# wuliwei9278/primalCR

Hardware: AMD Instinct MI355X
Metric: pairwise-comparisons/sec (higher is better)
Workload: dtype f32; 1 GPU; ml1m-shaped PrimalCR++ -k 100 -l 5000 (configs[1]); 6040 users x 3952 items, 939809 ratings, 131347247 ordered pairs; 1 step = 1 outer iteration (V step + U step); solver=PrimalCR++, rank=100, parallelism=user-sharded x1, accumulation=f64, storage=f32

## Files before the change

primalcr_amd/csrc/pcr_classes.h:

```cpp
#pragma once
#include <cstdio>
#include <cstring>

#include "pcr_dev.h"
#include "pcr_kernels.h"
#include "pcr_gram.h"

struct Bin {
    int block = 64;
    bool big = false;
    int K = 1;
    int ugrid = 0;
    int scratch_ofs = 0;
    int cap = 0;
    int limit = 0;
    int rcap = 0;
    int unr = 4;
    bool gram = false;
    int wcap = 0;
    int sym = 0;
    int max_lev = 0;
    int64_t nnz = 0;
    std::vector<int32_t> users;
    DBuf<int32_t> d_users;
};
static const int BIN_LIMIT[3] = {128, 512, 4096};
static const int BIN_BLOCK[4] = {64, 256, 512, 512};
static const int GRAM_DEFAULT_CAP = 0;

static void length_order(const std::vector<int64_t>& uptr, int64_t nu, std::vector<int32_t>& order) {
    order.resize((size_t)nu);
    int64_t maxlen = 0;
    for (int64_t u = 0; u < nu; ++u) maxlen = std::max(maxlen, uptr[u + 1] - uptr[u]);
    if (maxlen > ((int64_t)1 << 24)) {
        for (int64_t u = 0; u < nu; ++u) order[u] = (int32_t)u;
        std::stable_sort(order.begin(), order.end(), [&](int32_t a, int32_t b) { return (uptr[a + 1] - uptr[a]) > (uptr[b + 1] - uptr[b]); });
        return;
    }
    std::vector<int64_t> start((size_t)maxlen + 2, 0);
    for (int64_t u = 0; u < nu; ++u) start[(size_t)(maxlen - (uptr[u + 1] - uptr[u])) + 1]++;
    for (int64_t l = 0; l <= maxlen; ++l) start[(size_t)l + 1] += start[(size_t)l];
    for (int64_t u = 0; u < nu; ++u) order[(size_t)start[(size_t)(maxlen - (uptr[u + 1] - uptr[u]))]++] = (int32_t)u;
}
static void make_bins(const std::vector<int64_t>& uptr, int64_t nu, const std::vector<int64_t>* runofs, std::vector<Bin>& out,
                      const std::vector<int32_t>& order,
                      const std::vector<int>& limits = {BIN_LIMIT[0], BIN_LIMIT[1], BIN_LIMIT[2]},
                      const std::vector<int>& blocks = {BIN_BLOCK[0], BIN_BLOCK[1], BIN_BLOCK[2], BIN_BLOCK[3]}) {
    const int nb = (int)limits.size() + 1;
    out.clear();
    out.resize(nb);
    for (int b = 0; b < nb; ++b) { out[b].block = blocks[b]; out[b].big = (b == nb - 1); out[b].limit = b < nb - 1 ? limits[b] : 0; }
    for (int64_t q = 0; q < nu; ++q) {
        const int32_t u = order[(size_t)q];
        int64_t len = uptr[u + 1] - uptr[u];
        int b = 0;
        while (b < nb - 1 && len > limits[b]) ++b;
        out[b].users.push_back(u);
        out[b].nnz += len;
        out[b].cap = std::max<int>(out[b].cap, (int)len);
        if (runofs) out[b].max_lev = std::max<int>(out[b].max_lev, (int)((*runofs)[u + 1] - (*runofs)[u]) - 1);
    }
}
static std::string pname(const char* cls, const Bin& b) {
    if (b.gram) return std::string(cls) + "/gram" + std::to_string(b.block) + "." + std::to_string(b.limit);
    std::string s = std::string(cls) + "/" + std::to_string(b.block);
    if (!strcmp(cls, "ustep") && b.limit) s += "." + std::to_string(b.limit);
    const bool us = !strcmp(cls, "ustep");
    return s + (b.big ? "g" : "") + (b.K > 1 ? "c" : "") + (us && b.K == 1 && b.unr == 8 ? "l" : "") + (us && b.block == 64 && b.rcap > 0 ? "r" : "") +
           (b.sym ? "#" + std::to_string(b.sym) : "");
}

template <typename T>
static int pick_sweep_wave_cap(const std::vector<int64_t>& uptr, int64_t nu, const std::vector<int32_t>& by_len, int ncu) {
    int sweep_wave_cap = 256;
    {
        std::vector<int64_t> lens(nu);
        for (int64_t q = 0; q < nu; ++q) { const int32_t u = by_len[(size_t)(nu - 1 - q)]; lens[q] = uptr[u + 1] - uptr[u]; }
        const int64_t max_lds = std::upper_bound(lens.begin(), lens.end(), (int64_t)4096) - lens.begin();
        const int64_t cap_b = max_lds > 0 ? lens[max_lds - 1] : 0;
        double best = 0.0;
        for (int c : {256, 320, 384, 448, 512}) {
            const int64_t n_wave = std::upper_bound(lens.begin(), lens.end(), (int64_t)c) - lens.begin();
            const int64_t n_blk = std::max<int64_t>(0, max_lds - n_wave);
            const size_t wave_lds = 8 * ((size_t)c * sizeof(T) + (size_t)(c + 1) * 8 + 64);
            const size_t blk_lds = n_blk > 0 ? (size_t)cap_b * sizeof(T) + (size_t)(cap_b + 1) * 8 + 1024 : 0;
            const int per_cu = (int)std::max<size_t>(1, std::min<size_t>(4, ((size_t)160 << 10) / std::max<size_t>(1, std::max(wave_lds, blk_lds))));
            const double rounds = (double)(cdiv(n_wave, 8) + n_blk) / ((double)ncu * per_cu);
            const double cost = std::max(rounds, 1.0) * (1.0 + c / 1024.0);
            if (best == 0.0 || cost < best) { best = cost; sweep_wave_cap = c; }
        }
    }
    return sweep_wave_cap;
}

struct UstepLayoutIn {
    const std::vector<int64_t>& uptr;
    int64_t nu;
    const std::vector<int64_t>& run_ofs;
    const std::vector<int32_t>& by_len;
    int max_levels;
    int ld, nchunk, ncu;
    const std::string& ubins;
    int ustep_gram, ustep_mode, cluster_k, cluster_users, window_cache, ustep_win_lds;
};
struct UstepLayout {
    std::vector<Bin> ubins;
    size_t nsmall = 0;
// ... 157 lines not shown
```

primalcr_amd/csrc/pcr_eval.h:

```cpp
#pragma once
#include "pcr_prims.h"
#include "pcr_vside.h"

template <typename T>
static inline size_t eval_bytes(int cap) { return carve_bytes(cap, sizeof(T)) + carve_bytes(cap, 8) + carve_bytes(cap, 4); }

template <typename T, int BLOCK, bool BIG>
__global__ __launch_bounds__(BLOCK) void k_eval(const int64_t* __restrict__ uptr, const int32_t* __restrict__ item,
                                                const double* __restrict__ val, const double* __restrict__ gain,
                                                const double* __restrict__ idcg, const double* __restrict__ disc, int ndcg_k,
                                                const int32_t* __restrict__ users, int nusers, const T* __restrict__ U,
                                                const T* __restrict__ Vm, Geo geo, double* __restrict__ out4, int cap,
                                                char* scratch, size_t stride) {
    extern __shared__ __attribute__((aligned(16))) char smem[];
    Carver small(smem);
    T* vecT = small.take<T>(geo.ld);
    double* red = small.take<double>(BLOCK / PCR_WAVE + 1);
    T* wmax = small.take<T>(BLOCK / PCR_WAVE + 1);
    int* widx = small.take<int>(BLOCK / PCR_WAVE + 1);
    Carver big(BIG ? scratch + (size_t)blockIdx.x * stride : small.p);
    T* sc = big.take<T>(cap);
    double* vv = big.take<double>(cap);
    int32_t* itm = big.take<int32_t>(cap);
    const int tid = threadIdx.x, lane = tid & 63, wid = tid >> 6;
// ... 86 lines not shown
    double* red = small.take<double>(BLOCK / PCR_WAVE + 1);
    int* rs = small.take<int>(rs_cap);
    Carver big(BIG ? scratch + (size_t)blockIdx.x * stride : small.p);
    T* key = big.take<T>(cap_pad);
    LI* li = big.take<LI>(cap_pad);
    int32_t* itm = big.take<int32_t>(cap);
    const int tid = threadIdx.x;
    for (int ui = blockIdx.x; ui < nusers; ui += gridDim.x) {
        const int u = users[ui];
        const int64_t s0 = uptr[u];
        const int n = (int)(uptr[u + 1] - s0);
        const int nlev = (int)(erunofs[u + 1] - erunofs[u]) - 1;
        if (n == 0) {
            if (tid == 0) { out4[4 * (size_t)u] = 0.0; out4[4 * (size_t)u + 1] = 0.0; out4[4 * (size_t)u + 2] = 0.0; out4[4 * (size_t)u + 3] = 0.0; }
            continue;
        }
        for (int t = tid; t < geo.ld; t += BLOCK) vecT[t] = U[(size_t)u * geo.ld + t];
        for (int p = tid; p < n; p += BLOCK) itm[p] = item[s0 + p];
        for (int l = tid; l <= nlev; l += BLOCK) rs[l] = erunstart[erunofs[u] + l];
        __syncthreads();
        block_sddmm<T, BLOCK>(Vm, vecT, itm, n, key, geo);
        const int npad = next_pow2(n);
        for (int p = tid; p < npad; p += BLOCK) {
            if (p < n) li[p] = LiOps<LI>::pack(elvl[s0 + p], (unsigned)p);
            else { li[p] = LiOps<LI>::pack(0xFFFFu, (unsigned)p); key[p] = (T)0; }
        }
        __syncthreads();
        bitonic_sort<T, LI, BLOCK, true, !BIG>(key, li, npad, n);
        double bad = 0.0;
        for (int p = tid; p < n; p += BLOCK) {
            const int lev = (int)LiOps<LI>::lev(li[p]);
            const T sa = key[p];
            unsigned long long cnt = 0;
            for (int l = lev + 1; l < nlev; ++l) cnt += (unsigned long long)(ubound(key, rs[l], rs[l + 1], sa) - rs[l]);
            bad += (double)cnt;
        }
        const double badsum = block_sum<BLOCK>(bad, red);
        const double npairs = 0.5 * (double)n * (double)(n - 1);
        if (tid < PCR_WAVE) {
            const int lane = tid;
            int cur = (lane < nlev) ? rs[lane + 1] - 1 : -1;
            const int lo = (lane < nlev) ? rs[lane] : 0;
            const int nowk = n < ndcg_k ? n : ndcg_k;
            double dcg = 0.0;
            for (int k = 0; k < nowk; ++k) {
                const bool have = (lane < nlev) && cur >= lo;
                T best = have ? key[cur] : (T)0;
                int bi = have ? (int)LiOps<LI>::idx(li[cur]) : -1;
                int owner = lane;
#pragma unroll
                for (int off = 32; off > 0; off >>= 1) {
                    const T ob = __shfl_xor(best, off);
                    const int oi = __shfl_xor(bi, off);
                    const int oo = __shfl_xor(owner, off);
                    if (oi >= 0 && (bi < 0 || ob > best || (ob == best && oi < bi))) { best = ob; bi = oi; owner = oo; }
                }
                if (lane == owner) cur -= 1;
                dcg += gain[s0 + bi] * disc[k];
            }
            if (lane == 0) {
                out4[4 * (size_t)u] = (npairs > 0.0) ? badsum / npairs : 0.0;
                out4[4 * (size_t)u + 1] = (npairs > 0.0) ? 1.0 : 0.0;
                out4[4 * (size_t)u + 2] = dcg / idcg[u];
                out4[4 * (size_t)u + 3] = 1.0;
            }
        }
        __syncthreads();
    }
}

__global__ __launch_bounds__(PCR_EW_BLOCK) void k_sum4_stage1(const double* __restrict__ in, int64_t n, int per_block,
                                                               double* __restrict__ part) {
    __shared__ double red[PCR_EW_BLOCK / PCR_WAVE + 1];
    const int64_t lo = (int64_t)blockIdx.x * per_block;
    const int64_t hi = (lo + per_block < n) ? lo + per_block : n;
    double a[4] = {0.0, 0.0, 0.0, 0.0};
    for (int64_t i = lo + threadIdx.x; i < hi; i += PCR_EW_BLOCK)
        for (int c = 0; c < 4; ++c) a[c] += in[4 * i + c];
    for (int c = 0; c < 4; ++c) {
        const double s = block_sum<PCR_EW_BLOCK>(a[c], red);
        if (threadIdx.x == 0) part[4 * blockIdx.x + c] = s;
    }
}
template <typename T>
__global__ __launch_bounds__(PCR_EW_BLOCK) void k_obj3(const double* __restrict__ objx, const double* __restrict__ objx2, int64_t nx,
                                                        const T* __restrict__ a, int64_t na, const T* __restrict__ b, int64_t nb,
                                                        double* __restrict__ part, const double* __restrict__ wx = nullptr) {
    __shared__ double red[PCR_EW_BLOCK / PCR_WAVE + 1];
    const int64_t G = gridDim.x, blk = blockIdx.x;
    double s[4] = {0.0, 0.0, 0.0, 0.0};
    { const int64_t per = (nx + G - 1) / G, lo = blk * per, hi = lo + per < nx ? lo + per : nx;
      if (wx) for (int64_t i = lo + threadIdx.x; i < hi; i += PCR_EW_BLOCK) s[0] += wx[i] * objx[i];
      else for (int64_t i = lo + threadIdx.x; i < hi; i += PCR_EW_BLOCK) s[0] += objx[i];
      if (objx2) for (int64_t i = lo + threadIdx.x; i < hi; i += PCR_EW_BLOCK) s[3] += objx2[i]; }
    { const int64_t per = (na + G - 1) / G, lo = blk * per, hi = lo + per < na ? lo + per : na;
      for (int64_t i = lo + threadIdx.x; i < hi; i += PCR_EW_BLOCK) { const double v = (double)a[i]; s[1] += v * v; } }
    if (b) { const int64_t per = (nb + G - 1) / G, lo = blk * per, hi = lo + per < nb ? lo + per : nb;
      for (int64_t i = lo + threadIdx.x; i < hi; i += PCR_EW_BLOCK) { const double v = (double)b[i]; s[2] += v * v; } }
    for (int c = 0; c < 4; ++c) {
        const double t = block_sum<PCR_EW_BLOCK>(s[c], red);
        if (threadIdx.x == 0) part[4 * blk + c] = t;
    }
}
__global__ __launch_bounds__(PCR_EW_BLOCK) void k_fin4(const double* __restrict__ part, int nblk, double* __restrict__ out,
                                                        unsigned long long* cnt = nullptr, double* cnt_out = nullptr, int nzero = 0,
                                                        int keep1 = 1) {
    __shared__ double red[PCR_EW_BLOCK / PCR_WAVE + 1];
    for (int c = 0; c < 4; ++c) {
        double x = 0.0;
        for (int i = threadIdx.x; i < nblk; i += PCR_EW_BLOCK) x += part[4 * i + c];
        x = block_sum<PCR_EW_BLOCK>(x, red);
        if (threadIdx.x == 0) out[c] = (c == 1 && !keep1) ? 0.0 : x;
    }
    if (cnt) {
        if (threadIdx.x == 0) { cnt_out[0] = (double)cnt[0]; cnt_out[1] = (double)cnt[1]; cnt_out[2] = (double)cnt[3]; cnt_out[3] = (double)cnt[2]; }
        __syncthreads();
        for (int i = threadIdx.x; i < nzero; i += PCR_EW_BLOCK) cnt[i] = 0ull;
    }
}

__global__ __launch_bounds__(256) void k_gain_from_levels(const int64_t* __restrict__ uptr, const uint16_t* __restrict__ lvl,
                                                          const int64_t* __restrict__ runofs, const double* __restrict__ lgain,
                                                          double* __restrict__ gain, int64_t nu) {
    const int lane = threadIdx.x & 63;
    for (int64_t u = (int64_t)blockIdx.x * 4 + (threadIdx.x >> 6); u < nu; u += (int64_t)gridDim.x * 4) {
        const int64_t a = uptr[u], b = uptr[u + 1];
        const double* g = lgain + runofs[u];
        for (int64_t z = a + lane; z < b; z += 64) gain[z] = g[lvl[z]];
    }
}

template <typename T>
__global__ __launch_bounds__(256) void k_predict(const T* __restrict__ U, const T* __restrict__ Vm, const int32_t* __restrict__ user,
                                                 const int32_t* __restrict__ item, int64_t n, Geo geo, double* __restrict__ pred) {
    typedef typename VecOf<T>::type V;
    constexpr int VEC = VecOf<T>::N;
    const int G = geo.G, g = threadIdx.x & (G - 1);
    const int64_t z = ((int64_t)blockIdx.x * 256 + threadIdx.x) / G;
    if (z >= n) return;
    const T* up = U + (size_t)user[z] * geo.ld;
    const T* vp = Vm + (size_t)item[z] * geo.ld;
    T acc = (T)0;
    for (int ch = g; ch < geo.nchunk; ch += G)
        acc += vdot(*reinterpret_cast<const V*>(up + ch * VEC), *reinterpret_cast<const V*>(vp + ch * VEC));
    for (int off = G >> 1; off > 0; off >>= 1) acc += __shfl_xor(acc, off);
    if (g == 0) pred[z] = (double)acc;
}
```

primalcr_amd/csrc/pcr_gram.h:

```cpp
#pragma once
#include "pcr_kernels.h"

typedef float pcr_f32x16 __attribute__((ext_vector_type(16)));
typedef double pcr_f64x4 __attribute__((ext_vector_type(4)));

template <typename T> struct GramMfma;
template <> struct GramMfma<float> {
    static constexpr int TS = 32, KS = 2, NACC = 16;
    typedef pcr_f32x16 acc_t;
    static __device__ __forceinline__ acc_t mma(float a, float b, acc_t c) { return __builtin_amdgcn_mfma_f32_32x32x2f32(a, b, c, 0, 0, 0); }
    static __device__ __forceinline__ int crow(int j, int l) { return (j & 3) + 8 * (j >> 2) + 4 * (l >> 5); }
    static __device__ __forceinline__ int ccol(int l) { return l & 31; }
};
template <> struct GramMfma<double> {
    static constexpr int TS = 16, KS = 4, NACC = 4;
    typedef pcr_f64x4 acc_t;
    static __device__ __forceinline__ acc_t mma(double a, double b, acc_t c) { return __builtin_amdgcn_mfma_f64_16x16x4f64(a, b, c, 0, 0, 0); }
    static __device__ __forceinline__ int crow(int j, int l) { return (l >> 4) + 4 * j; }
    static __device__ __forceinline__ int ccol(int l) { return l & 15; }
};

template <int BLOCK, int NV>
__device__ __forceinline__ void block_sums(double (&v)[NV], double* red) {
#pragma unroll
    for (int i = 0; i < NV; ++i) v[i] = wave_sum(v[i]);
    if (BLOCK == PCR_WAVE) return;
    const int wid = threadIdx.x >> 6, lane = threadIdx.x & 63;
    __syncthreads();
    if (lane == 0) {
#pragma unroll
        for (int i = 0; i < NV; ++i) red[wid * NV + i] = v[i];
    }
    __syncthreads();
#pragma unroll
    for (int i = 0; i < NV; ++i) {
        double t = 0.0;
#pragma unroll
        for (int w = 0; w < BLOCK / PCR_WAVE; ++w) t += red[w * NV + i];
        v[i] = t;
    }
}

template <typename T>
__host__ __device__ static inline size_t gram_img_bytes(int cap, int nchp) {
    const size_t x = (size_t)cap * nchp * 16, k = (size_t)cap * cap * sizeof(T);
    return x > k ? x : k;
}
template <typename T>
static inline size_t gram_bytes(int cap, int cap_pad, int rs_cap, int ld, int nchp, int block) {
    return 3 * carve_bytes(ld, 8) + carve_bytes((size_t)(block / PCR_WAVE) * 8 + 8, 8) + carve_bytes((size_t)(block / PCR_WAVE) * ld, 8) +
           carve_bytes(gram_img_bytes<T>(cap, nchp), 1) + 12 * carve_bytes(cap, 8) + carve_bytes(cap, sizeof(T)) + carve_bytes(cap_pad, sizeof(T)) +
           carve_bytes(cap, 2) + carve_bytes(cap, 4) + carve_bytes(cap_pad, 4) + carve_bytes(cap + 1, 8) + carve_bytes(rs_cap, 4);
}

template <typename T, int BLOCK>
__global__ __launch_bounds__(BLOCK) void k_ustep_gram(Shard<T> S, Geo geo, const int32_t* __restrict__ users, int nusers,
                                                      T* __restrict__ U, const T* __restrict__ Vm, double lambda, double stepsize0,
                                                      int cg_max, double cg_tol, int strict, int solver1, int cap, int cap_pad,
                                                      int rs_cap, int nchp, unsigned long long* counters, int count_rows) {
    typedef GramMfma<T> MM;
    typedef uint32_t LI;
    constexpr int VEC = VecOf<T>::N, NW = BLOCK / PCR_WAVE;
    extern __shared__ __attribute__((aligned(16))) char smem[];
    Carver cv(smem);
    const int ld = geo.ld;
    double* uvec = cv.take<double>(ld);
    double* unew = cv.take<double>(ld);
    double* tmpv = cv.take<double>(ld);
    double* red = cv.take<double>((size_t)NW * 8 + 8);
    double* wbuf = cv.take<double>((size_t)NW * ld);
    char* img = cv.take<char>(gram_img_bytes<T>(cap, nchp));
    double* md = cv.take<double>(cap);
    double* ad = cv.take<double>(cap);
    double* kd = cv.take<double>(cap);
    double* ar = cv.take<double>(cap);
    double* kr = cv.take<double>(cap);
    double* ap = cv.take<double>(cap);
    double* kp = cv.take<double>(cap);
    double* ah = cv.take<double>(cap);
    double* kh = cv.take<double>(cap);
    double* cc = cv.take<double>(cap);
    double* kc = cv.take<double>(cap);
    double* bb = cv.take<double>(cap);
    T* ms0 = cv.take<T>(cap);
    T* key = cv.take<T>(cap_pad);
    uint16_t* lv0 = cv.take<uint16_t>(cap);
    int32_t* itm = cv.take<int32_t>(cap);
    LI* li = cv.take<LI>(cap_pad);
    double* Sx = cv.take<double>(cap + 1);
    int* rs = cv.take<int>(rs_cap);
    const int tid = threadIdx.x, lane = tid & 63, wid = tid >> 6;
    const int lstride = nchp * VEC;
    T* X = reinterpret_cast<T*>(img);
    T* K = reinterpret_cast<T*>(img);

#ifdef PCR_USTEP_PROF
    long long prof_[12] = {0, 0, 0, 0, 0, 0, 0, 0, 0, 0, 0, 0}, tprev_ = clock64();
    const long long tstart_ = tprev_;
#endif
    for (int ui = blockIdx.x; ui < nusers; ui += gridDim.x) {
        const int u = users[ui];
        const int64_t s0 = S.uptr[u];
        const int n = (int)(S.uptr[u + 1] - s0);
        const int nlev = (int)(S.runofs[u + 1] - S.runofs[u]) - 1;
        for (int t = tid; t < ld; t += BLOCK) { uvec[t] = (double)U[(size_t)u * ld + t]; unew[t] = uvec[t]; }
        for (int p = tid; p < n; p += BLOCK) { ms0[p] = S.ms[s0 + p]; md[p] = (double)ms0[p]; lv0[p] = S.slvl[s0 + p]; itm[p] = S.sitem[s0 + p]; }
        for (int l = tid; l <= nlev; l += BLOCK) rs[l] = S.runstart[S.runofs[u] + l];
        __syncthreads();
        UPROF(0);
        if (n > 0) stage_rows<T, BLOCK>(Vm, itm, 0, n, X, geo, nchp);
        block_excl_scan<BLOCK>([&](int i) { return md[i]; }, Sx, n, red);
        const bool win = S.ws != 0;
        for (int p = tid; p < n; p += BLOCK)
            cc[p] = win ? sweep_coeff_cached<T>(S, (size_t)s0 + p, Sx, rs, nlev, lv0[p], md[p], 1.0)
                        : sweep_coeff<T>(ms0, Sx, rs, nlev, lv0[p], ms0[p], md[p], 1.0, strict);
        UPROF(1);
        asm volatile("s_waitcnt vmcnt(0)" ::: "memory");
        __syncthreads();
        UPROF(7);
        for (int p = tid; p < n; p += BLOCK) {
            const T* xr = X + (size_t)p * lstride;
            double acc0 = 0.0;
            for (int t = 0; t < ld; ++t) acc0 += (double)xr[t] * uvec[t];
            md[p] = acc0;
// ... 183 lines not shown
```

primalcr_amd/csrc/pcr_host.cpp:

```cpp
#include "pcr_host.h"

#include <algorithm>
#include <atomic>
#include <cerrno>
#include <climits>
#include <cstdint>
#include <cmath>
#include <cstdio>
#include <cstdlib>
#include <cstring>
#include <exception>
#include <functional>
#include <limits>
#include <memory>
#include <mutex>
#include <numeric>
#include <random>
#include <thread>
#include <fcntl.h>
#include <sys/mman.h>
#include <sys/stat.h>
#include <unistd.h>

static thread_local std::string g_err;
// ... 213 lines not shown
}

static int check_test_ids(int64_t d2, int64_t tnnz, const int32_t* tuser, const int32_t* titem, int threads) {
    const int T = pieces_for(tnnz, threads);
    std::vector<int64_t> bad((size_t)T, -1);
    run_pieces(tnnz, T, [&](int t, int64_t lo, int64_t hi) {
        for (int64_t z = lo; z < hi; ++z)
            if (titem[z] < 0 || titem[z] >= d2 || tuser[z] < 0) { bad[(size_t)t] = z; return; }
    });
    for (int64_t b : bad)
        if (b >= 0) {
            pcr_set_error("test rating " + std::to_string(b) + " has user/item id outside the meta dimensions");
            return PCR_ERR_ARG;
        }
    return PCR_OK;
}

extern "C" int pcr_dataset_from_triplets(int64_t d1, int64_t d2, int64_t nnz, const int32_t* user,
                                         const int32_t* item, const double* val, int64_t tnnz,
                                         const int32_t* tuser, const int32_t* titem, const double* tval,
                                         pcr_dataset** out) {
    if (!out || d1 < 0 || d2 < 0 || nnz < 0 || tnnz < 0 || (nnz > 0 && (!user || !item || !val)) ||
        (tnnz > 0 && (!tuser || !titem || !tval))) {
        pcr_set_error("pcr_dataset_from_triplets: bad argument");
        return PCR_ERR_ARG;
    }
    if (d1 > kMaxDim || d2 > kMaxDim) { pcr_set_error("pcr_dataset_from_triplets: more than 2^31 - 2 users or items"); return PCR_ERR_UNSUPPORTED; }
    return guarded("pcr_dataset_from_triplets", [&]() -> int {
        std::unique_ptr<pcr_dataset> ds(new pcr_dataset());
        const int threads = pcr_host_threads();
        int rc = build_train_csr(d1, d2, nnz, user, item, val, ds->train, threads, false);
        if (rc != PCR_OK) return rc;
        rc = check_test_ids(d2, tnnz, tuser, titem, threads);
        if (rc != PCR_OK) return rc;
        keep_raw_test(*ds, d1, tnnz, tuser, titem, tval);
        build_test_csr(d1, d2, tnnz, tuser, titem, tval, ds->test, threads, false);
        ds->tnnz_file = tnnz;
        *out = ds.release();
        return PCR_OK;
    });
}

extern "C" int pcr_dataset_from_csr(int64_t d1, int64_t d2, const int64_t* index, const int32_t* item, const double* val,
                                    const int64_t* tindex, const int32_t* titem, const double* tval, pcr_dataset** out) {
    if (!out || d1 < 0 || d2 < 0 || !index || index[0] != 0 || (tindex && tindex[0] != 0)) {
        pcr_set_error("pcr_dataset_from_csr: bad argument");
        return PCR_ERR_ARG;
    }
    const int64_t nnz = index[d1], tnnz = tindex ? tindex[d1] : 0;
    if (nnz < 0 || tnnz < 0 || (nnz > 0 && (!item || !val)) || (tnnz > 0 && (!titem || !tval))) {
        pcr_set_error("pcr_dataset_from_csr: bad argument");
        return PCR_ERR_ARG;
    }
    for (int64_t u = 0; u < d1; ++u) {
        if (index[u + 1] < index[u] || (tindex && tindex[u + 1] < tindex[u])) { pcr_set_error("pcr_dataset_from_csr: index not monotone"); return PCR_ERR_ARG; }
        for (int64_t z = index[u]; z < index[u + 1]; ++z)
            if (item[z] < 0 || item[z] >= d2 || (z > index[u] && item[z] <= item[z - 1])) {
                pcr_set_error("pcr_dataset_from_csr: user " + std::to_string(u) + ": item ids must be ascending and inside [0, d2)");
                return PCR_ERR_ARG;
            }
    }
    for (int64_t z = 0; z < tnnz; ++z)
        if (titem[z] < 0 || titem[z] >= d2) { pcr_set_error("pcr_dataset_from_csr: test item id outside [0, d2)"); return PCR_ERR_ARG; }
    if (d1 > kMaxDim || d2 > kMaxDim) { pcr_set_error("pcr_dataset_from_csr: more than 2^31 - 2 users or items"); return PCR_ERR_UNSUPPORTED; }
    return guarded("pcr_dataset_from_csr", [&]() -> int {
        std::unique_ptr<pcr_dataset> ds(new pcr_dataset());
        ds->train.d1 = ds->test.d1 = d1; ds->train.d2 = ds->test.d2 = d2;
        ds->train.index.assign(index, index + d1 + 1);
        ds->train.item.assign(item, item + nnz);
        ds->train.val.assign(val, val + nnz);
        if (tindex) ds->test.index.assign(tindex, tindex + d1 + 1); else ds->test.index.assign(d1 + 1, 0);
        ds->test.item.assign(titem, titem + tnnz);
        ds->test.val.assign(tval, tval + tnnz);
        ds->tnnz_file = tnnz;
        *out = ds.release();
        return PCR_OK;
    });
}

#include <map>
static std::map<std::string, std::string>& tune_table() { static thread_local std::map<std::string, std::string> t; return t; }
static const char* const TUNE_KEYS[] = {"ustep_mode", "cluster_k", "cluster_users", "ubins", "ustep_gram", "spmm_tiles", "spmm_chunk", "sddmm_csc",
                                        "lanes", "pipeline", "window_cache", "prepare_merged", "resort_window", "allreduce_chunks", "p2p_ll",
                                        "p2p_timeout_ms", "p2p_queue_budget", "count_rows", "debug", "win16", "ustep_win_lds", "plan_key64", "ustep_newton", "vblock_users", "recommend_select", "ranks_batch_users", "sample_threads", "rerank_lds", "ridge_form", "nnls_form", "itemfold_table_bytes", "fault_cluster_member", "fault_p2p_skip", "fault_p2p_coarse", nullptr};
extern "C" int pcr_tune(const char* key, const char* value) {
    if (!key) { pcr_set_error("pcr_tune: null key"); return PCR_ERR_ARG; }
    bool known = false;
    for (const char* const* k = TUNE_KEYS; *k; ++k) known = known || !strcmp(*k, key);
    if (!known) { pcr_set_error(std::string("pcr_tune: unknown key '") + key + "'"); return PCR_ERR_ARG; }
    if (value) tune_table()[key] = value; else tune_table().erase(key);
    return PCR_OK;
}
bool pcr_tune_get(const char* key, std::string* out) {
    auto it = tune_table().find(key);
    if (it == tune_table().end()) return false;
    if (out) *out = it->second;
    return true;
}
int pcr_tune_int(const char* key, int dflt) {
    std::string v;
    return pcr_tune_get(key, &v) ? atoi(v.c_str()) : dflt;
}


struct TextFile {
    const char* p = nullptr;
    size_t len = 0;
    void* map = nullptr;
    size_t map_len = 0;
    pcr_vec<char> heap;
    ~TextFile() { if (map) munmap(map, map_len); }
    int open(const std::string& path) {
        const int fd = ::open(path.c_str(), O_RDONLY | O_CLOEXEC);
        if (fd < 0) { pcr_set_error("can't open " + path + ": " + strerror(errno)); return PCR_ERR_IO; }
        struct stat sb;
        if (fstat(fd, &sb) == 0 && S_ISREG(sb.st_mode) && sb.st_size > 0) {
            void* m = mmap(nullptr, (size_t)sb.st_size, PROT_READ, MAP_PRIVATE, fd, 0);
            if (m != MAP_FAILED) {
                (void)madvise(m, (size_t)sb.st_size, MADV_WILLNEED);
                map = m; map_len = (size_t)sb.st_size; p = static_cast<const char*>(m); len = map_len;
                ::close(fd);
                return PCR_OK;
            }
        }
        size_t cap = (size_t)1 << 20, got = 0;
        heap.resize(cap);
        for (;;) {
            const ssize_t n = ::read(fd, heap.data() + got, cap - got);
            if (n < 0) { if (errno == EINTR) continue; ::close(fd); pcr_set_error("can't read " + path + ": " + strerror(errno)); return PCR_ERR_IO; }
            if (n == 0) break;
            got += (size_t)n;
            if (got == cap) { cap *= 2; heap.resize(cap); }
        }
        ::close(fd);
        p = heap.data(); len = got;
        return PCR_OK;
    }
};

struct SlowCopy {
    char buf[512];
    size_t n;
    SlowCopy(const char* p, const char* end) { n = std::min<size_t>(sizeof(buf) - 1, (size_t)(end - p)); memcpy(buf, p, n); buf[n] = 0; }
};

static inline bool parse_one(const char*& p, const char* end, int32_t& u, int32_t& it, double& v) {
    auto skip_ws = [&]() { while (p < end && (*p == ' ' || *p == '\t' || *p == '\n' || *p == '\r')) ++p; };
    auto parse_uint = [&](long& out) -> bool {
        skip_ws();
        const char* s = p;
        long x = 0;
        while (p < end && *p >= '0' && *p <= '9') { if (x < ((long)1 << 40)) x = x * 10 + (*p - '0'); ++p; }
        if (p == s || (p < end && (*p == '.' || *p == '-' || *p == '+' || *p == 'e' || *p == 'E'))) { p = s; return false; }
        out = x;
        return true;
    };
    const char* save = p;
    long a, b;
    if (parse_uint(a) && parse_uint(b)) {
        skip_ws();
        const char* s = p;
        bool neg = false;
        if (p < end && (*p == '-' || *p == '+')) { neg = *p == '-'; ++p; }
        long ip = 0; int nd = 0;
        while (p < end && *p >= '0' && *p <= '9' && nd < 15) { ip = ip * 10 + (*p - '0'); ++p; ++nd; }
        bool simple = nd > 0 || (p < end && *p == '.');
        double val = (double)ip;
// ... 1503 lines not shown
```

primalcr_amd/csrc/pcr_prims.h:

```cpp
#pragma once
#include <hip/hip_runtime.h>
#include <stdint.h>

#define PCR_WAVE 64

template <typename T> struct VecOf;
template <> struct VecOf<float>  { typedef float4 type;  static constexpr int N = 4; };
template <> struct VecOf<double> { typedef double2 type; static constexpr int N = 2; };

__device__ __forceinline__ float  vdot(const float4& a, const float4& b)  { return a.x * b.x + a.y * b.y + a.z * b.z + a.w * b.w; }
__device__ __forceinline__ double vdot(const double2& a, const double2& b) { return a.x * b.x + a.y * b.y; }
__device__ __forceinline__ float  velem(const float4& a, int e)  { return e == 0 ? a.x : e == 1 ? a.y : e == 2 ? a.z : a.w; }
__device__ __forceinline__ double velem(const double2& a, int e) { return e == 0 ? a.x : a.y; }

struct Geo { int r, ld, nchunk, G; };
__device__ __forceinline__ size_t row_off(int row, const Geo& geo) { return (size_t)((unsigned long long)(unsigned)row * (unsigned)geo.ld); }

template <typename T>
struct Shard {
    int64_t nu, nnz;
    int d2;
    const int64_t* uptr;
    const int32_t* item;
    const uint16_t* lvl;
    const int64_t* runofs;
    const int32_t* runstart;
    T* ms;
    int32_t* sitem;
    uint16_t* slvl;
    int32_t* sidx;
    double* objp;
    double* objr;
    void* win;
    int ws, w16;
    int resort_d, prev_valid;
    unsigned char* rhint;
    const double* uw = nullptr;
    const double* ulam = nullptr;
};


__device__ __forceinline__ int dpp_xor1(int v) { return __builtin_amdgcn_mov_dpp(v, 0xB1, 0xF, 0xF, true); }
__device__ __forceinline__ int dpp_xor2(int v) { return __builtin_amdgcn_mov_dpp(v, 0x4E, 0xF, 0xF, true); }
__device__ __forceinline__ int swz_xor4(int v) { return __builtin_amdgcn_ds_swizzle(v, 0x101F); }
__device__ __forceinline__ int swz_xor8(int v) { return __builtin_amdgcn_ds_swizzle(v, 0x201F); }
__device__ __forceinline__ int perm_xor16(int v) {
    const auto r = __builtin_amdgcn_permlane16_swap(v, v, false, false);
    return (threadIdx.x & 16) ? (int)r[0] : (int)r[1];
}
__device__ __forceinline__ int perm_xor32(int v) {
    const auto r = __builtin_amdgcn_permlane32_swap(v, v, false, false);
    return (threadIdx.x & 32) ? (int)r[0] : (int)r[1];
}
template <int OFF> __device__ __forceinline__ int lane_xor_i(int v) {
    static_assert(OFF == 1 || OFF == 2 || OFF == 4 || OFF == 8 || OFF == 16 || OFF == 32, "power of two below 64");
    return OFF == 1 ? dpp_xor1(v) : OFF == 2 ? dpp_xor2(v) : OFF == 4 ? swz_xor4(v) : OFF == 8 ? swz_xor8(v) : OFF == 16 ? perm_xor16(v) : perm_xor32(v);
}
template <int OFF> __device__ __forceinline__ float lane_xor(float v) { return __int_as_float(lane_xor_i<OFF>(__float_as_int(v))); }
template <int OFF> __device__ __forceinline__ double lane_xor(double v) {
    return __hiloint2double(lane_xor_i<OFF>(__double2hiint(v)), lane_xor_i<OFF>(__double2loint(v)));
}
__device__ __forceinline__ float lane_xor1(float v) { return __int_as_float(dpp_xor1(__float_as_int(v))); }
__device__ __forceinline__ float lane_xor2(float v) { return __int_as_float(dpp_xor2(__float_as_int(v))); }
__device__ __forceinline__ double lane_xor1(double v) {
    return __hiloint2double(dpp_xor1(__double2hiint(v)), dpp_xor1(__double2loint(v)));
}
__device__ __forceinline__ double lane_xor2(double v) {
    return __hiloint2double(dpp_xor2(__double2hiint(v)), dpp_xor2(__double2loint(v)));
}

template <int CTRL, int ROWMASK> __device__ __forceinline__ double dpp_zero_fill(double v) {
    const int hi = __builtin_amdgcn_update_dpp(0, __double2hiint(v), CTRL, ROWMASK, 0xF, false);
    const int lo = __builtin_amdgcn_update_dpp(0, __double2loint(v), CTRL, ROWMASK, 0xF, false);
    return __hiloint2double(hi, lo);
}
__device__ __forceinline__ double wave_incl_scan(double v) {
    v += dpp_zero_fill<0x111, 0xF>(v);
    v += dpp_zero_fill<0x112, 0xF>(v);
    v += dpp_zero_fill<0x114, 0xF>(v);
    v += dpp_zero_fill<0x118, 0xF>(v);
    v += dpp_zero_fill<0x142, 0xA>(v);
    v += dpp_zero_fill<0x143, 0xC>(v);
    return v;
}
__device__ __forceinline__ double lane63(double v) {
    return __hiloint2double(__builtin_amdgcn_readlane(__double2hiint(v), 63), __builtin_amdgcn_readlane(__double2loint(v), 63));
}

__device__ __forceinline__ double wave_sum(double v) {
    v += lane_xor<32>(v); v += lane_xor<16>(v); v += lane_xor<8>(v); v += lane_xor<4>(v);
    v += lane_xor2(v);
    v += lane_xor1(v);
    return v;
}

__device__ __forceinline__ void wave_sync() {
    __builtin_amdgcn_fence(__ATOMIC_RELEASE, "wavefront");
    __builtin_amdgcn_wave_barrier();
    __builtin_amdgcn_fence(__ATOMIC_ACQUIRE, "wavefront");
}

template <int BLOCK> __device__ __forceinline__ void bsync() { if (BLOCK == PCR_WAVE) wave_sync(); else __syncthreads(); }
template <int BLOCK> __device__ __forceinline__ int btid() { return BLOCK == PCR_WAVE ? (int)(threadIdx.x & 63) : (int)threadIdx.x; }

template <int BLOCK>
__device__ __forceinline__ double block_sum(double v, double* red) {
    v = wave_sum(v);
    if (BLOCK == PCR_WAVE) return v;
    const int wid = threadIdx.x >> 6, lane = threadIdx.x & 63;
    __syncthreads();
    if (lane == 0) red[wid] = v;
    __syncthreads();
    double t = 0.0;
#pragma unroll
    for (int w = 0; w < BLOCK / PCR_WAVE; ++w) t += red[w];
    return t;
}

template <int BLOCK, class F>
__device__ __forceinline__ void block_excl_scan(F f, double* out, int n, double* red) {
    const int tid = btid<BLOCK>(), lane = tid & 63, wid = tid >> 6;
    double carry = 0.0;
    for (int base = 0; base < n; base += BLOCK) {
        const int i = base + tid;
        const double v = (i < n) ? f(i) : 0.0;
        const double inc = wave_incl_scan(v);
        double woff = 0.0, total;
        if (BLOCK > PCR_WAVE) {
            __syncthreads();
            if (lane == 63) red[wid] = inc;
            __syncthreads();
            total = 0.0;
#pragma unroll
            for (int w = 0; w < BLOCK / PCR_WAVE; ++w) {
                double x = red[w];
                if (w < wid) woff += x;
                total += x;
            }
        } else {
            total = lane63(inc);
        }
        if (i < n) out[i] = carry + woff + inc - v;
        carry += total;
    }
    if (tid == 0) out[n] = carry;
    bsync<BLOCK>();
}

template <typename LI> struct LiOps;
template <> struct LiOps<uint32_t> {
    static constexpr int SH = 16;
    static __device__ __forceinline__ uint32_t pack(unsigned lv, unsigned idx) { return (lv << 16) | idx; }
    static __device__ __forceinline__ unsigned lev(uint32_t x) { return x >> 16; }
    static __device__ __forceinline__ unsigned idx(uint32_t x) { return x & 0xFFFFu; }
};
template <> struct LiOps<uint64_t> {
    static constexpr int SH = 32;
    static __device__ __forceinline__ uint64_t pack(unsigned lv, unsigned idx) { return ((uint64_t)lv << 32) | idx; }
    static __device__ __forceinline__ unsigned lev(uint64_t x) { return (unsigned)(x >> 32); }
    static __device__ __forceinline__ unsigned idx(uint64_t x) { return (unsigned)(x & 0xFFFFFFFFu); }
};

template <typename T, typename LI, int BLOCK, bool TIE = false, bool INLDS = true>
__device__ __forceinline__ void bitonic_sort(T* key, LI* li, int npad, int n) {
    const int tid = btid<BLOCK>();
    for (int k = 2; k <= npad; k <<= 1) {
        for (int j = k >> 1; j > 0; j >>= 1) {
            for (int t = tid; t < (npad >> 1); t += BLOCK) {
                const int i = ((t & ~(j - 1)) << 1) | (t & (j - 1));
                const int l = (j == (k >> 1)) ? (i ^ (k - 1)) : (i | j);
                if (l >= n) continue;
                T ka = key[i], kb = key[l];
                LI la = li[i], lb = li[l];
                unsigned va = LiOps<LI>::lev(la), vb = LiOps<LI>::lev(lb);
                bool b_lt_a = (vb < va) || (vb == va && kb < ka);
                if (TIE && va == vb && ka == kb) b_lt_a = LiOps<LI>::idx(lb) > LiOps<LI>::idx(la);
                if (b_lt_a) { key[i] = kb; key[l] = ka; li[i] = lb; li[l] = la; }
            }
            const int jnext = j > 1 ? (j >> 1) : k;
            const bool last = (j == 1 && k == npad);
            if (INLDS && !last && j <= 64 && jnext <= 64) wave_sync(); else bsync<BLOCK>();
        }
    }
}

#ifdef PCR_RESORT_STAT
__device__ unsigned long long g_resort_stat[4];
#endif
template <typename T, typename LI, int BLOCK, class LevF>
__device__ __forceinline__ bool resort_window_d(T* key, LI* li, LevF levf, const int* rs, int n, int* tmp, T* key2, int D, int* flag) {
    static_assert(sizeof(LI) <= sizeof(T) || sizeof(LI) == 4, "li is permuted through key2's bytes");
    const int tid = btid<BLOCK>();
#pragma unroll 1
    for (int p = tid; p < n; p += BLOCK) tmp[p] = -1;
    if (BLOCK > PCR_WAVE && tid == 0) *flag = 0;
    bsync<BLOCK>();
#pragma unroll 1
    for (int p = tid; p < n; p += BLOCK) {
        const int lev = levf(p);
// ... 432 lines not shown
```

primalcr_amd/csrc/pcr_solver.hip:

```cpp
#include <hip/hip_runtime.h>
#include <rccl/rccl.h>

#include <algorithm>
#include <chrono>
#include <cmath>
#include <cstdio>
#include <cstring>
#include <memory>
#include <string>
#include <vector>

#include "pcr_host.h"
#include "pcr_dev.h"
#include "pcr_kernels.h"
#include "pcr_gram.h"
#include "pcr_newton.h"
#include "pcr_vblock.h"
#include "pcr_p2p.h"

#define NCCLCHK(expr)                                                                          \
    do {                                                                                       \
        ncclResult_t e_ = (expr);                                                              \
        if (e_ != ncclSuccess) {                                                               \
            pcr_set_error(std::string(#expr) + ": " + ncclGetErrorString(e_));                 \
            return PCR_ERR_COMM;                                                               \
        }                                                                                      \
    } while (0)
#include "pcr_plan.h"
#include "pcr_plan_dev.h"

#include "pcr_classes.h"

struct Tune {
    int lanes = 0, spmm_chunk = 0, spmm_tiles = 0, sddmm_csc = -1, ustep_mode = 0, cluster_k = 4, cluster_users = 0, window_cache = 1,
        prepare_merged = -1, pipeline = 1, debug = 0, fault_cluster_member = 0, ustep_gram = -1, count_rows = 0, allreduce_chunks = 0,
        resort_window = 8, p2p_ll = 16, p2p_timeout_ms = 20000, p2p_queue_budget = 0, fault_p2p_skip = 0, fault_p2p_coarse = 0, win16 = 1, ustep_win_lds = 1, plan_key64 = 0, ustep_newton = 0, vblock_users = 0, recommend_select = 1;
    std::string ubins;
    void read() {
        lanes = pcr_tune_int("lanes", 0); spmm_chunk = pcr_tune_int("spmm_chunk", 0); spmm_tiles = pcr_tune_int("spmm_tiles", 0);
        sddmm_csc = pcr_tune_int("sddmm_csc", -1); ustep_mode = pcr_tune_int("ustep_mode", 0); cluster_k = pcr_tune_int("cluster_k", 4);
        cluster_users = pcr_tune_int("cluster_users", 0); window_cache = pcr_tune_int("window_cache", 1);
        prepare_merged = pcr_tune_int("prepare_merged", -1);
        pipeline = pcr_tune_int("pipeline", 1); debug = pcr_tune_int("debug", 0); fault_cluster_member = pcr_tune_int("fault_cluster_member", 0);
        ustep_gram = pcr_tune_int("ustep_gram", -1); count_rows = pcr_tune_int("count_rows", 0);
        allreduce_chunks = pcr_tune_int("allreduce_chunks", 0);
        resort_window = pcr_tune_int("resort_window", 8); p2p_ll = pcr_tune_int("p2p_ll", 16);
        p2p_timeout_ms = pcr_tune_int("p2p_timeout_ms", 20000); fault_p2p_skip = pcr_tune_int("fault_p2p_skip", 0);
        fault_p2p_coarse = pcr_tune_int("fault_p2p_coarse", 0); p2p_queue_budget = pcr_tune_int("p2p_queue_budget", 0);
        win16 = pcr_tune_int("win16", 1); ustep_win_lds = pcr_tune_int("ustep_win_lds", 1); plan_key64 = pcr_tune_int("plan_key64", 0); ustep_newton = pcr_tune_int("ustep_newton", 0); vblock_users = pcr_tune_int("vblock_users", 0);
        recommend_select = pcr_tune_int("recommend_select", 1);
        ubins.clear(); pcr_tune_get("ubins", &ubins);
    }
};

template <typename T>
struct Solver final : pcr_solver {
    pcr_params prm;
    Tune tune;
    int rank = 0, nranks = 1;
    int64_t d1 = 0, d2 = 0, tnnz_file = 0;
    Geo geo;
    hipStream_t st = nullptr;
    static constexpr int NSIDE = 12;
    hipStream_t side[NSIDE] = {};
    hipEvent_t ev_fork = nullptr;
    hipStream_t hi = nullptr;
    hipEvent_t ev_hi = nullptr;
    static constexpr int MAXLANE = 8;
    hipStream_t lane[MAXLANE] = {};
    hipEvent_t ev_lane[MAXLANE] = {};
    int nlane = 1;
    int pipe_lanes = 0;
    bool hi_on_solver_pipe = false;
    std::vector<hipStream_t> hi_spare;
    ncclComm_t comm = nullptr;
    std::unique_ptr<P2PComm> p2p;
    bool single() const { return (nranks == 1 && !comm && !p2p) || local_only; }
    int ncu = 256;

    Shard<T> sh;
    DBuf<int64_t> d_uptr, d_runofs;
    DBuf<int32_t> d_sidx;
    DBuf<double> d_objr;
    DBuf<int32_t> d_item, d_c2r, d_runstart, d_sitem, d_cuser, d_crow, d_ruser, d_slot_base, d_item_slot, d_chunk_ptr, d_slot_id;
    DBuf<int2> d_blk_chunks;
    DBuf<int32_t> d_blk_user, d_cpos_dense;
    DBuf<unsigned char> d_excl;
    int vblock_nbp = 0;
    DBuf<int32_t> d_newton_users;
    DBuf<double> d_dir;
    DBuf<char> d_newton_scratch;
    int newton_n = 0, newton_cap = 0, newton_rs = 0, newton_grid = 0;
    size_t newton_stride = 0;
    DBuf<int32_t> d_cuf;
    int spmm_blocks = 0, spmm_tiles = 1;
    int n_rng = 1;
    std::vector<int64_t> rng_item;
    std::vector<int> rng_blk;
    hipStream_t ar_st = nullptr;
    std::vector<hipEvent_t> ev_rng;
    hipEvent_t ev_ar = nullptr;
    bool sddmm_csc = false;
    DBuf<T> d_slab;
    bool sweep_pf4 = false;
    int spmm_chunk = 128;
    int sddmm_tile = 0;
    DBuf<uint16_t> d_lvl, d_slvl;
    DBuf<unsigned char> d_rhint;
    DBuf<uint16_t> d_win;
    DBuf<T> d_ms, d_c, d_mcsr, d_b;
    DBuf<double> d_objp;
    std::vector<Bin> bins;
    std::vector<Bin> sbins;
    std::vector<Bin> pbins;
    std::vector<Bin> ubins;
    unsigned* bar_p = nullptr;
    size_t bar_n = 0;
    DBuf<char> d_xch;
    DBuf<unsigned long long> d_rowcnt;
    size_t xch_stride = 0;
    int max_clusters = 1;
    struct EvalSet {
        int64_t nnz = 0;
        DBuf<int64_t> uptr;
        DBuf<int32_t> item;
        DBuf<double> val, gain, idcg, disc;
        DBuf<uint16_t> elvl;
        DBuf<int64_t> erunofs;
        DBuf<int32_t> erunstart;
        int max_raw_levels = 0;
        std::vector<Bin> bins;
        std::vector<int64_t> h_uptr;
        std::vector<double> h_val;
        std::vector<int64_t> h_runofs;
        std::vector<int32_t> h_cnt;
        std::vector<double> h_lgain;
// ... 320 lines not shown
        }
        return PCR_OK;
    }
    int shard_bounds(const pcr_dataset* ds, int64_t shard_first, int64_t d1_total, HostShard& H) {
        const PcrCsr& X = ds->train;
        d1 = X.d1; d2 = X.d2; tnnz_file = ds->tnnz_file;
        if (prm.k < 1) { pcr_set_error("rank k must be >= 1"); return PCR_ERR_ARG; }
        if (d2 >= (int64_t)1 << 31 || d1 >= (int64_t)1 << 31) { pcr_set_error("d1/d2 must fit in int32"); return PCR_ERR_UNSUPPORTED; }
        geo.r = prm.k;
        geo.ld = (prm.k + 3) & ~3;
        geo.nchunk = geo.ld / VecOf<T>::N;
        geo.G = std::min(64, host_pow2(geo.nchunk));

        if (shard_first >= 0) {
            if (d1_total < shard_first + X.d1 || d1_total >= (int64_t)1 << 31) { pcr_set_error("pcr_solver_create_shard: the shard does not fit the job's user range"); return PCR_ERR_ARG; }
            if (ds->test.d1 != X.d1) { pcr_set_error("pcr_solver_create_shard: train and test user counts differ"); return PCR_ERR_ARG; }
            first_user = shard_first; n_users = X.d1; d1 = d1_total;
        } else {
            std::vector<int64_t> bounds(nranks + 1);
            RC(pcr_partition_users(X.index.data(), d1, nranks, bounds.data()));
            first_user = bounds[rank];
            n_users = bounds[rank + 1] - bounds[rank];
            H.u0 = first_user;
        }
        nnz_local = X.index[H.u0 + n_users] - X.index[H.u0];
        if (nnz_local >= ((int64_t)1 << 31) - 1) { pcr_set_error("more than 2^31 ratings on one GPU"); return PCR_ERR_UNSUPPORTED; }
        return PCR_OK;
    }
    int pick_blocked_users(const HostShard& H) {
        const std::vector<int64_t>& uptr = H.uptr;
        const int64_t nu = n_users;
        if (tune.vblock_users > 0 && nu > 0) {
            const int64_t blk_cap = std::min<int64_t>(tune.vblock_users, (((int64_t)1 << 30) / 4 / std::max<int64_t>(d2, 1)) & ~(int64_t)31);
            std::vector<int32_t> blk;
            std::vector<int32_t> cpos;
            for (int64_t q = 0; q < nu && (int64_t)blk.size() < blk_cap; ++q) {
                const int32_t u = H.by_len[(size_t)q];
                if ((uptr[u + 1] - uptr[u]) * 16 < d2) break;
                const size_t row = blk.size() * (size_t)d2;
                cpos.resize(row + (size_t)d2, -1);
                bool dup = false;
                for (int64_t z = uptr[u]; z < uptr[u + 1] && !dup; ++z) {
                    int32_t& slot = cpos[row + (size_t)H.item[z]];
                    dup = slot != -1;
                    slot = (int32_t)z;
                }
                if (dup) {
                    cpos.resize(row);
                    if (tune.debug) fprintf(stderr, "[pcr] blocked-user V step: user %d rates an item twice -- left in the sparse plan\n", (int)u);
                    continue;
                }
                blk.push_back(u);
            }
            if (!blk.empty()) {
                vblock_nbp = ((int)blk.size() + 31) & ~31;
                std::vector<unsigned char> excl((size_t)nu, 0);
                cpos.resize((size_t)vblock_nbp * (size_t)d2, -1);
                for (int32_t u : blk) excl[(size_t)u] = 1;
                blk.resize((size_t)vblock_nbp, -1);
                RC(d_blk_user.upload(blk, st)); RC(d_cpos_dense.upload(cpos, st)); RC(d_excl.upload(excl, st));
                if (tune.debug) fprintf(stderr, "[pcr] blocked-user V step: %d users (padded to %d) x %lld items through the dense kernels\n",
                                        (int)std::count(excl.begin(), excl.end(), 1), vblock_nbp, (long long)d2);
            }
        }
        return PCR_OK;
    }
    int adopt_plan(const HostShard& H) {
        SpmmPlan P;
        const SpmmPlanIn plan_in{H.uptr, H.item, n_users, nnz_local, d2, geo.ld, geo.G, ncu, sizeof(T), tune.spmm_chunk, tune.spmm_tiles, vblock_nbp ? 0 : tune.allreduce_chunks};
        RC(build_plan(plan_in, P));
        spmm_chunk = P.chunk; n_rng = P.n_rng; rng_item = P.rng_item; rng_blk = P.rng_blk; spmm_blocks = P.blocks; spmm_tiles = P.ntiles;
        if (n_rng > 1) {
            HIPCHK(hipStreamCreateWithFlags(&ar_st, hipStreamNonBlocking));
            HIPCHK(hipEventCreateWithFlags(&ev_ar, hipEventDisableTiming));
            ev_rng.resize(n_rng);
            for (auto& e : ev_rng) HIPCHK(hipEventCreateWithFlags(&e, hipEventDisableTiming));
        }
        RC(d_slab.alloc(std::max<size_t>(P.slab_rows, 1) * geo.ld));
        sddmm_csc = (size_t)d2 * geo.ld * sizeof(T) > ((size_t)32 << 20) && spmm_tiles >= 8;
        if (tune.sddmm_csc >= 0) sddmm_csc = tune.sddmm_csc != 0;
        if (vblock_nbp) sddmm_csc = true;
        return PCR_OK;
    }
    int setup_vside_classes(const HostShard& H) {
        const int64_t nu = n_users;
        make_bins(H.uptr, nu, &H.lv.run_ofs, bins, H.by_len);
        for (auto& b : bins) RC(b.d_users.upload(b.users, st));
        const int sweep_wave_cap = pick_sweep_wave_cap<T>(H.uptr, nu, H.by_len, ncu);
        if (tune.debug) fprintf(stderr, "[pcr] sweep wave cap %d\n", sweep_wave_cap);
        make_bins(H.uptr, nu, &H.lv.run_ofs, sbins, H.by_len, {std::min(sweep_wave_cap, 4095), 4096}, {64, 512, 512});
        for (auto& b : sbins) RC(b.d_users.upload(b.users, st));
        const int prep_wave_cap = 256;
        make_bins(H.uptr, nu, &H.lv.run_ofs, pbins, H.by_len, {prep_wave_cap, 4096}, {64, 512, 512});
        for (auto& b : pbins) RC(b.d_users.upload(b.users, st));
        sweep_pf4 = true;
        return PCR_OK;
    }
    int setup_ustep_classes(const HostShard& H) {
        UstepLayout L;
        std::string err;
        const int rc = ustep_class_layout<T>({H.uptr, n_users, H.lv.run_ofs, H.by_len, H.lv.max_levels, geo.ld, geo.nchunk, ncu, tune.ubins, tune.ustep_gram,
                                              tune.ustep_mode, tune.cluster_k, tune.cluster_users, tune.window_cache, tune.ustep_win_lds}, L, err);
        if (rc != PCR_OK) { pcr_set_error(err); return rc; }
        ubins = std::move(L.ubins);
        u_big_blocks = L.u_big_blocks; max_clusters = L.max_clusters; xch_stride = L.xch_stride; bar_n = L.bar_n;
        sh.ws = L.ws;
        for (auto& b : ubins) RC(b.d_users.upload(b.users, st));
        RC(d_xch.alloc(xch_stride * (size_t)max_clusters * ubins.size()));
        RC(d_rowcnt.alloc(ubins.size()));
        HIPCHK(hipMemset(d_rowcnt.p, 0, std::max<size_t>(ubins.size(), 1) * sizeof(unsigned long long)));
        return PCR_OK;
    }
    int setup_newton(const HostShard& H) {
        const int64_t nu = n_users;
        if (tune.ustep_newton && geo.ld <= NEWTON_MAX_LD) {
            std::vector<int32_t> nus_list;
            for (int64_t q = 0; q < nu; ++q) {
                const int32_t u = H.by_len[(size_t)q];
                const int64_t len = H.uptr[u + 1] - H.uptr[u];
                if (len >= 1 && len <= NEWTON_MAX_N) { nus_list.push_back(u); newton_cap = std::max<int>(newton_cap, (int)len); }
            }
            newton_n = (int)nus_list.size();
            newton_rs = H.lv.max_levels + 2;
            RC(d_newton_users.upload(nus_list, st));
            RC(d_dir.alloc((size_t)std::max<int64_t>(nu, 1) * geo.ld));
            const int ldp = (geo.ld + 15) & ~15;
            newton_grid = std::max(1, std::min(newton_n, 2 * ncu));
            newton_stride = (((size_t)newton_cap + 1) * ldp * sizeof(double) + 255) & ~(size_t)255;
            RC(d_newton_scratch.alloc(newton_stride * (size_t)newton_grid));
#ifndef PCR_NO_OPTIONAL_KERNELS
            HIPCHK(hipFuncSetAttribute((const void*)k_unewton<T>, hipFuncAttributeMaxDynamicSharedMemorySize, 160 * 1024));
#endif
            if (tune.debug) fprintf(stderr, "[pcr] exact-Newton U step: %d of %lld users through the explicit Hessian (<= %d ratings)\n", newton_n, (long long)nu, NEWTON_MAX_N);
        }
        return PCR_OK;
    }
    int setup_state(const HostShard& H) {
        const int64_t nu = n_users;
        RC(d_lvl.upload(H.lv.level, st));
        RC(d_runofs.upload(H.lv.run_ofs, st)); RC(d_runstart.upload(H.lv.run_start, st));
        RC(d_ms.alloc(nnz_local)); RC(d_sitem.alloc(nnz_local)); RC(d_slvl.alloc(nnz_local));
        RC(d_c.alloc(nnz_local)); RC(d_objp.alloc(nu)); RC(d_mcsr.alloc(nnz_local)); RC(d_b.alloc(nnz_local));
        sh.nu = nu; sh.nnz = nnz_local; sh.d2 = (int)d2;
        sh.uptr = d_uptr.p; sh.item = d_item.p; sh.lvl = d_lvl.p;
        sh.runofs = d_runofs.p; sh.runstart = d_runstart.p;
        sh.ms = d_ms.p; sh.sitem = d_sitem.p; sh.slvl = d_slvl.p; sh.objp = d_objp.p;
        RC(d_sidx.alloc(nnz_local)); RC(d_objr.alloc(nu));
        sh.sidx = d_sidx.p; sh.objr = d_objr.p;
        sh.resort_d = std::max(0, std::min(tune.resort_window, 64));
        sh.prev_valid = 0;
        RC(d_rhint.alloc(std::max<int64_t>(nu, 1)));
        HIPCHK(hipMemsetAsync(d_rhint.p, 0, std::max<int64_t>(nu, 1), st));
        sh.rhint = d_rhint.p;
        {
            int64_t longest = 0;
            for (int64_t u = 0; u < nu; ++u) longest = std::max(longest, H.uptr[u + 1] - H.uptr[u]);
            sh.w16 = (longest < 65536 && tune.win16) ? 1 : 0;
        }
        RC(d_win.alloc((size_t)nnz_local * sh.ws * (sh.w16 ? 1 : 2)));
        sh.win = d_win.p;
        return PCR_OK;
    }
    int build_eval_set(int w, const PcrCsr& E, const HostShard& H) {
        EvalSet& es = ev[w];
        const PcrLevels& lv = H.lv;
        const int64_t nu = n_users, ds_u0 = H.u0;
        const int64_t a = E.index[ds_u0], b = E.index[ds_u0 + nu];
        es.nnz = b - a;
        es.h_uptr.resize(nu + 1);
        for (int64_t u = 0; u <= nu; ++u) es.h_uptr[u] = E.index[ds_u0 + u] - a;
        if (w == 1) {
            RC(es.uptr.upload(es.h_uptr, st)); RC(es.item.upload_n(E.item.data() + a, (size_t)es.nnz));
            h_test_item.assign(E.item.begin() + a, E.item.begin() + b); h_test_val.assign(E.val.begin() + a, E.val.begin() + b);
        }
// ... 302 lines not shown
        const int ngrp = 256 / geo.G, span = ngrp * tile;
        const int grid = cdiv(nnz_local, span);
        hipLaunchKernelGGL((k_sddmm<T, 256>), dim3(grid), dim3(256), (size_t)span * 8, st, Umat, M, d_ruser.p, rows, nnz_local, out, geo, tile, skip,
                           (const int32_t*)nullptr, (const int2*)nullptr, (const int32_t*)nullptr);
        HIPCHK(hipGetLastError());
        return PCR_OK;
    }
    bool sddmm_by_tiles() const { return sddmm_csc; }
    int launch_sddmm_csc(const T* A, T* out, const int* skip) {
        if (nnz_local == 0) return PCR_OK;
        ProfScope ps(&prof, "sddmm", st);
        const int span = (256 / geo.G) * spmm_chunk;
        hipLaunchKernelGGL((k_sddmm<T, 256>), dim3(spmm_blocks), dim3(256), (size_t)span * 8, st, A, d_U.p, d_crow.p, d_cuser.p, nnz_local, out, geo,
                           spmm_chunk, skip, d_c2r.p, d_blk_chunks.p, d_chunk_ptr.p);
        HIPCHK(hipGetLastError());
        return PCR_OK;
    }

    bool prepare_is_single_launch() const {
        const bool merged = tune.prepare_merged >= 0 ? tune.prepare_merged != 0 : nnz_local < (int64_t)4000000;
        return merged && !pbins[0].users.empty() && !pbins[1].users.empty();
    }
    int launch_prepare(const T* Vm) {
        RC(launch_sddmm(Vm, d_item.p, d_mcsr.p));
        const Shard<T>& shp = sh;
        auto fn = [&](Bin& b, hipStream_t q) {
            const int nus = (int)b.users.size();
            const int cap_pad = b.big ? host_pow2(b.cap) : b.cap, rsc = b.max_lev + 2;
            const size_t bigb = prepare_bytes<T>(b.cap, cap_pad, rsc, b.big ? 8 : 4);
            const size_t lds = small_common(b.block) + (b.big ? 0 : bigb);
            const int grid = b.big ? std::min(nus, scratch_blocks) : nus;
#define LP(BL, BG) hipLaunchKernelGGL((k_prepare<T, BL, BG>), dim3(grid), dim3(BL), lds, q, shp, geo, b.d_users.p, nus, d_mcsr.p, b.cap, cap_pad, rsc, d_scratch.p, scratch_stride, strict())
            if (b.big) LP(512, true);
            else if (b.block == 64) LP(64, false);
            else if (b.block == 256) LP(256, false);
            else LP(512, false);
#undef LP
        };
        Bin &ba = pbins[0], &bb = pbins[1];
        if (prepare_is_single_launch()) {
            const int na = (int)ba.users.size(), nb = (int)bb.users.size();
            const int cpa = ba.cap, cpb = bb.cap, rsa = ba.max_lev + 2, rsb = bb.max_lev + 2;
            const size_t wb = (small_common(64) + prepare_bytes<T>(ba.cap, cpa, rsa, 4) + 15) & ~(size_t)15;
            const int wbs = 512, wpb = wbs / 64;
            const size_t lds = std::max(wb * wpb, small_common(wbs) + prepare_bytes<T>(bb.cap, cpb, rsb, 4));
            {
                ProfScope ps(&prof, "prepare/all", st, ba.nnz + bb.nnz, (int64_t)(na + nb));
                hipLaunchKernelGGL((k_prepare_all<T, 512>), dim3(nb + cdiv(na, wpb)), dim3(512), lds, st, shp, ba.d_users.p, na, ba.cap, cpa, rsa, wb,
                                   bb.d_users.p, nb, bb.cap, cpb, rsb, nb, d_mcsr.p, strict());
            }
            if (!pbins[2].users.empty()) { ProfScope ps(&prof, pname("prepare", pbins[2]), st, pbins[2].nnz, (int64_t)pbins[2].users.size()); fn(pbins[2], st); }
            HIPCHK(hipGetLastError());
            have_sorted = true;
            sh.prev_valid = 1;
            return PCR_OK;
        }
        RC(for_bins(bins, "prepare", fn));
        have_sorted = true;
        sh.prev_valid = 1;
        return PCR_OK;
    }

    int launch_vsweep(bool hv, const T* A, const int* skip = nullptr) {
        if (hv) { if (sddmm_by_tiles()) RC(launch_sddmm_csc(A, d_b.p, skip)); else RC(launch_sddmm(A, d_sitem.p, d_b.p, skip)); }
        if (hv && vblock_nbp) {
            ProfScope ps(&prof, "vblock_b", st);
            const int64_t tiles = (int64_t)(vblock_nbp / GramMfma<T>::TS) * cdiv(d2, GramMfma<T>::TS);
#ifndef PCR_NO_OPTIONAL_KERNELS
            hipLaunchKernelGGL((k_vblock_b<T>), dim3((unsigned)cdiv(tiles, 4)), dim3(256), 0, st, d_U.p, A, d_blk_user.p, vblock_nbp, d_cpos_dense.p, d2, geo, d_b.p, skip);
#endif
            HIPCHK(hipGetLastError());
        }
        return launch_sweeps(hv, skip, hv && sddmm_by_tiles());
    }
    int launch_sweeps(bool hv, const int* skip, bool b_csr = false) {
        const int bc = (b_csr ? 1 : 0) | (sweep_pf4 ? 2 : 0);
        const bool two = hv && !sh.ws;
        const bool wt = sh.uw != nullptr;
        auto fn = [&](Bin& b, hipStream_t q) {
            const int nus = (int)b.users.size();
            const int rsc = b.max_lev + 2;
            if (b.block == 64) {
                const size_t wb = (vsweep_wave_bytes<T>(b.cap, rsc, two) + 15) & ~(size_t)15;
#define LW(HV, WT) hipLaunchKernelGGL((k_vsweep_wave<T, HV, WT>), dim3(cdiv(nus, 4)), dim3(256), wb * 4, q, sh, b.d_users.p, nus, d_b.p, d_c.p, b.cap, rsc, wb, strict(), skip, bc)
                if (hv) { if (wt) LW(true, true); else LW(true, false); } else { if (wt) LW(false, true); else LW(false, false); }
#undef LW
                return;
            }
            const size_t bigb = vsweep_bytes<T>(b.cap, rsc, two);
            const size_t lds = small_common(b.block) + (b.big ? 0 : bigb);
            const int grid = b.big ? std::min(nus, scratch_blocks) : nus;
#define LV(BL, BG, HV) do { if (wt) LVW(BL, BG, HV, true); else LVW(BL, BG, HV, false); } while (0)
#define LVW(BL, BG, HV, WT) hipLaunchKernelGGL((k_vsweep<T, BL, BG, HV, WT>), dim3(grid), dim3(BL), lds, q, sh, geo, b.d_users.p, nus, d_b.p, d_c.p, b.cap, rsc, d_scratch.p, scratch_stride, strict(), skip, bc)
            if (hv) { if (b.big) LV(512, true, true); else LV(512, false, true); }
            else { if (b.big) LV(512, true, false); else LV(512, false, false); }
#undef LVW
#undef LV
        };
        Bin &ba = sbins[0], &bb = sbins[1];
        if (!ba.users.empty() && !bb.users.empty()) {
            const int na = (int)ba.users.size(), nb = (int)bb.users.size();
            const int rsa = ba.max_lev + 2, rsb = bb.max_lev + 2;
            const size_t wb = (vsweep_wave_bytes<T>(ba.cap, rsa, two) + 15) & ~(size_t)15;
            const int wbs = 512, wpb = wbs / 64;
            const size_t lds = std::max(wb * wpb, small_common(wbs) + vsweep_bytes<T>(bb.cap, rsb, two));
            const int grid = nb + cdiv(na, wpb);
            {
                ProfScope ps(&prof, std::string(hv ? "vhv" : "vgrad") + "/all", st, ba.nnz + bb.nnz, (int64_t)(na + nb));
#define LVA(HV, WBS, MW) do { if (wt) LVAW(HV, WBS, MW, true); else LVAW(HV, WBS, MW, false); } while (0)
#define LVAW(HV, WBS, MW, WT) hipLaunchKernelGGL((k_vsweep_all<T, HV, WBS, MW, WT>), dim3(grid), dim3(WBS), lds, st, sh, ba.d_users.p, na, ba.cap, rsa, wb, \
                                        bb.d_users.p, nb, bb.cap, rsb, nb, d_b.p, d_c.p, strict(), skip, bc)
                const bool dense = lds <= (size_t)40 * 1024;
                if (hv) { if (dense) { LVA(true, 512, 8); } else { LVA(true, 512, 1); } } else { if (dense) { LVA(false, 512, 8); } else { LVA(false, 512, 1); } }
#undef LVAW
#undef LVA
            }
            if (!sbins[2].users.empty()) { ProfScope ps(&prof, pname(hv ? "vhv" : "vgrad", sbins[2]), st, sbins[2].nnz, (int64_t)sbins[2].users.size()); fn(sbins[2], st); }
            HIPCHK(hipGetLastError());
            return PCR_OK;
        }
        RC(for_bins_seq(sbins, hv ? "vhv" : "vgrad", fn));
        return PCR_OK;
    }

    int fin_blocks() const { return (int)std::min<int64_t>(1024, cdiv(d2, 256 / geo.G)); }
    int launch_spmm_range(int r, T* out, const T* base, double beta, const int* skip, const T* dots_rr) {
        if (nnz_local > 0 && rng_blk[r + 1] > rng_blk[r]) {
            ProfScope ps(&prof, "spmm", st);
            hipLaunchKernelGGL((k_spmm<T, 256>), dim3(rng_blk[r + 1] - rng_blk[r]), dim3(256), 0, st, d_c.p, d_c2r.p, d_cuf.p,
                               d_chunk_ptr.p, d_slot_base.p, d_slot_id.p, d_blk_chunks.p + rng_blk[r], d_U.p, d_slab.p, geo, skip);
        }
        const int j0 = (int)rng_item[r], j1 = (int)rng_item[r + 1];
        if (j1 <= j0) return PCR_OK;
        const int grid = n_rng == 1 ? fin_blocks() : (int)std::min<int64_t>(1024, cdiv(j1 - j0, 256 / geo.G));
        ProfScope ps2(&prof, "spmm_fin", st);
        if (dots_rr) hipLaunchKernelGGL((k_spmm_fin<T, 256, true>), dim3(grid), dim3(256), 0, st, d_slab.p, d_item_slot.p, base, beta, j1, out, geo, skip, dots_rr, d_partA.p, j0);
        else hipLaunchKernelGGL((k_spmm_fin<T, 256, false>), dim3(grid), dim3(256), 0, st, d_slab.p, d_item_slot.p, base, beta, j1, out, geo, skip, (const T*)nullptr, (double*)nullptr, j0);
        return PCR_OK;
    }
    int launch_spmm(T* out, const T* base, double beta, const int* skip = nullptr, const T* dots_rr = nullptr) {
        const size_t n = (size_t)d2 * geo.ld;
        if (n_rng == 1) {
            RC(launch_spmm_range(0, out, base, beta, skip, dots_rr));
            if (vblock_nbp) {
                ProfScope ps(&prof, "vblock_hp", st);
                const int64_t tiles = (int64_t)cdiv(d2, GramMfma<T>::TS) * cdiv(geo.ld, GramMfma<T>::TS);
#ifndef PCR_NO_OPTIONAL_KERNELS
                hipLaunchKernelGGL((k_vblock_hp<T>), dim3((unsigned)cdiv(tiles, 4)), dim3(256), 0, st, d_U.p, d_c.p, d_blk_user.p, vblock_nbp, d_cpos_dense.p, d2, geo, out, skip);
#endif
            }
            HIPCHK(hipGetLastError());
            return allreduce_T(out, n);
        }
        const bool exch = !single();
        auto queue = [&](int r) -> int {
            RC(launch_spmm_range(r, out, base, beta, skip, nullptr));
            if (exch) HIPCHK(hipEventRecord(ev_rng[r], st));
            return PCR_OK;
        };
        RC(queue(0));
        for (int r = 0; r < n_rng; ++r) {
            if (r + 1 < n_rng) RC(queue(r + 1));
            if (!exch) continue;
            HIPCHK(hipStreamWaitEvent(ar_st, ev_rng[r], 0));
            const size_t lo = (size_t)rng_item[r] * geo.ld, hi = (size_t)rng_item[r + 1] * geo.ld;
            if (hi > lo) RC(allreduce_T(out + lo, hi - lo, ar_st));
        }
        if (exch) { HIPCHK(hipEventRecord(ev_ar, ar_st)); HIPCHK(hipStreamWaitEvent(st, ev_ar, 0)); }
        HIPCHK(hipGetLastError());
        return PCR_OK;
    }

    int allreduce_T(T* buf, size_t count, hipStream_t q = nullptr) {
        if (single()) return PCR_OK;
        if (!comm && !p2p) { pcr_set_error("nranks > 1 but neither pcr_solver_comm_init nor pcr_solver_comm_init_p2p was called"); return PCR_ERR_STATE; }
        if (!q) q = st;
        ProfScope ps(&prof, "allreduce", q);
        if (p2p) {
            if (!p2p->allreduce<T>(buf, count, q)) { pcr_set_error("p2p all-reduce: " + p2p->err); return PCR_ERR_COMM; }
            return PCR_OK;
        }
        NCCLCHK(ncclAllReduce(buf, buf, count, sizeof(T) == 4 ? ncclFloat : ncclDouble, ncclSum, comm, q));
        return PCR_OK;
    }
    int allreduce_f64(double* buf, size_t count) override {
        if (single()) return PCR_OK;
        if (!comm && !p2p) { pcr_set_error("nranks > 1 but neither pcr_solver_comm_init nor pcr_solver_comm_init_p2p was called"); return PCR_ERR_STATE; }
        ProfScope ps(&prof, "allreduce", st);
        if (p2p) {
            if (!p2p->allreduce<double>(buf, count, st, true)) { pcr_set_error("p2p all-reduce: " + p2p->err); return PCR_ERR_COMM; }
            return PCR_OK;
        }
        NCCLCHK(ncclAllReduce(buf, buf, count, ncclDouble, ncclSum, comm, st));
        return PCR_OK;
    }

    int reduce_sum(const double* in, int64_t n, int slot) {
        const int nb = (int)std::min<int64_t>(512, std::max<int64_t>(1, cdiv(n, 2048)));
        const int per = cdiv(std::max<int64_t>(n, 1), nb);
        hipLaunchKernelGGL(k_sum_stage1, dim3(nb), dim3(PCR_EW_BLOCK), 0, st, in, n, per, d_partA.p);
        hipLaunchKernelGGL(k_fin2, dim3(1), dim3(PCR_EW_BLOCK), 0, st, d_partA.p, nb, d_scal.p + slot);
        HIPCHK(hipGetLastError());
        return PCR_OK;
    }
    int norm2(const T* a, int64_t n, int slot) {
        const int nb = (int)std::min<int64_t>(512, std::max<int64_t>(1, cdiv(n, 4096)));
        const int per = cdiv(std::max<int64_t>(n, 1), nb);
        hipLaunchKernelGGL((k_dots<T>), dim3(nb), dim3(PCR_EW_BLOCK), 0, st, a, (const T*)nullptr, n, per, d_partB.p);
        hipLaunchKernelGGL(k_fin2, dim3(1), dim3(PCR_EW_BLOCK), 0, st, d_partB.p, nb, d_scal.p + slot);
        HIPCHK(hipGetLastError());
        return PCR_OK;
    }
    int sync_checked() {
        HIPCHK(hipStreamSynchronize(st));
        if (p2p && p2p->exchange_failed()) { pcr_set_error("p2p all-reduce: " + p2p->err); return PCR_ERR_COMM; }
        return PCR_OK;
    }
    int fetch_scal(int count) {
        HIPCHK(hipMemcpyAsync(h_scal, d_scal.p, std::max(count, 44) * sizeof(double), hipMemcpyDeviceToHost, st));
        return sync_checked();
    }

    int objective_sums(const double* objx, const T* Vm, bool with_u, int slot = 0, const double* objx2 = nullptr, bool after_ustep = false) {
        const int64_t nV = (int64_t)d2 * geo.ld, nU = (int64_t)n_users * geo.ld;
        const int nb = (int)std::min<int64_t>(512, std::max<int64_t>(1, cdiv(std::max(nV, nU), 4096)));
        hipLaunchKernelGGL((k_obj3<T>), dim3(nb), dim3(PCR_EW_BLOCK), 0, st, objx, objx2, n_users, Vm, nV, with_u ? d_U.p : (const T*)nullptr, nU, d_partA.p,
                           objx == d_objp.p ? sh.uw : (const double*)nullptr);
        const bool reduce = !single();
        const int keep1 = (!reduce || rank == 0) ? 1 : 0;
        if (after_ustep) hipLaunchKernelGGL(k_fin4, dim3(1), dim3(PCR_EW_BLOCK), 0, st, d_partA.p, nb, d_scal.p + slot, d_counters.p, d_scal.p + slot + 4, counter_words(), keep1);
        else hipLaunchKernelGGL(k_fin4, dim3(1), dim3(PCR_EW_BLOCK), 0, st, d_partA.p, nb, d_scal.p + slot, (unsigned long long*)nullptr, (double*)nullptr, 0, keep1);
        HIPCHK(hipGetLastError());
        RC(allreduce_f64(d_scal.p + slot, after_ustep ? 8 : 4));
        return PCR_OK;
    }
    int full_objective(const T* Vm, double* obj) {
        const bool need_u = !unorm_valid;
        RC(objective_sums(d_objp.p, Vm, need_u));
        RC(fetch_scal(8));
        if (need_u) { unorm2 = h_scal[2]; unorm_valid = true; }
        *obj = h_scal[0] + prm.lambda * (unorm2 + h_scal[1]) / 2.0;
        return PCR_OK;
    }

    int upload_mat(const double* H, int64_t rows, T* D) { return upload_rows<T>(st, geo.r, geo.ld, {{H, rows, D}}); }
    int download_mat(const T* D, int64_t rows, double* H) {
        const int64_t slab_rows = std::max<int64_t>(1, ((int64_t)64 << 20) / std::max(1, geo.r));
        DBuf<double> stage;
        RC(stage.alloc((size_t)std::min(rows, slab_rows) * geo.r));
        for (int64_t r0 = 0; r0 < rows; r0 += slab_rows) {
            const int64_t nr = std::min(slab_rows, rows - r0);
            hipLaunchKernelGGL((k_mat_out<T>), dim3((unsigned)std::min<int64_t>(1 << 16, cdiv(nr * geo.r, 256))), dim3(256), 0, st, D + r0 * geo.ld, stage.p, nr, geo.r, geo.ld);
            HIPCHK(hipGetLastError());
            HIPCHK(hipMemcpyAsync(H + r0 * geo.r, stage.p, (size_t)nr * geo.r * sizeof(double), hipMemcpyDeviceToHost, st));
            RC(sync_checked());
        }
        if (rows == 0) RC(sync_checked());
        return PCR_OK;
    }

    int set_factors(const double* U, const double* V, bool local) override {
        if (U) { RC(upload_mat(U + (local ? 0 : first_user * geo.r), n_users, d_U.p)); unorm_valid = false; }
        if (V) RC(upload_mat(V, d2, d_V.p));
        have_sorted = false; state_of_rejected_V = false;
        return PCR_OK;
    }
    DBuf<double> d_uw, d_ulam;
    int set_user_weights(const double* w, bool local) override {
        if (tune.ustep_newton != 0 || tune.ustep_gram > 0 || tune.vblock_users > 0) {
            pcr_set_error(std::string("pcr_solver_set_user_weights: this solver was created under pcr_tune \"") +
                          (tune.ustep_newton != 0 ? "ustep_newton" : tune.ustep_gram > 0 ? "ustep_gram" : "vblock_users") +
                          "\", whose kernels do not carry per-user weights");
            return PCR_ERR_UNSUPPORTED;
        }
        for (const Bin& b : ubins)
            if (b.gram) { pcr_set_error("pcr_solver_set_user_weights: the dual-form U-step class (k_ustep_gram) does not carry per-user weights"); return PCR_ERR_UNSUPPORTED; }
        std::vector<double> hw, hl;
        if (w) {
            const double* mine = w + (local ? 0 : first_user);
            hw.assign(mine, mine + n_users);
            hl.resize((size_t)n_users);
            for (int64_t u = 0; u < n_users; ++u) {
                if (!(hw[(size_t)u] > 0.0) || !std::isfinite(hw[(size_t)u])) {
                    pcr_set_error("pcr_solver_set_user_weights: the weight of user " + std::to_string(first_user + u) + " is not a finite number > 0");
                    return PCR_ERR_ARG;
                }
                hl[(size_t)u] = prm.lambda / hw[(size_t)u];
            }
        }
        RC(sync_checked());
        if (ustep_pending) RC(ustep_finish(nullptr, nullptr));
        start_sums_queued = false;
        if (w) {
            RC(d_uw.upload_n(hw.data(), hw.size()));
            RC(d_ulam.upload_n(hl.data(), hl.size()));
            sh.uw = d_uw.p; sh.ulam = d_ulam.p;
        } else {
            sh.uw = nullptr; sh.ulam = nullptr;
        }
        return PCR_OK;
    }
    int get_factors(double* U, double* V, bool local) override {
        if (U) RC(download_mat(d_U.p, n_users, U + (local ? 0 : first_user * geo.r)));
        if (V) RC(download_mat(d_V.p, d2, V));
        return PCR_OK;
    }

    int comp_m(double* m_out) override {
        T* mc = d_mcsr.p;
        RC(launch_prepare(d_V.p));
        if (m_out) {
            std::vector<T> tmp(nnz_local);
            if (nnz_local) HIPCHK(hipMemcpyAsync(tmp.data(), mc, nnz_local * sizeof(T), hipMemcpyDeviceToHost, st));
            HIPCHK(hipStreamSynchronize(st));
            for (int64_t z = 0; z < nnz_local; ++z) m_out[z] = (double)tmp[z];
        }
        return PCR_OK;
    }
    int need_sorted() const {
        if (!have_sorted) { pcr_set_error("call pcr_comp_m first (no sorted state for the current factors)"); return PCR_ERR_STATE; }
        return PCR_OK;
    }
    int objective(double* obj) override {
        RC(need_sorted());
        return full_objective(d_V.p, obj);
    }

    int device_gradient() {
        RC(launch_vsweep(false, nullptr));
        return launch_spmm(d_g.p, d_V.p, rank == 0 ? prm.lambda : 0.0);
    }
    int obtain_g(double* g) override {
        RC(need_sorted());
        RC(device_gradient());
        return download_mat(d_g.p, d2, g);
    }
    int device_hv(const T* pvec, T* out, const int* skip = nullptr, const T* dots_rr = nullptr) {
        RC(launch_vsweep(true, pvec, skip));
        return launch_spmm(out, pvec, rank == 0 ? prm.lambda : 0.0, skip, dots_rr);
    }
#ifdef PCR_PIPE_PROBE
    int pipe_probe() {
        if (sbins[0].users.empty() || sbins[1].users.empty() || n_rng != 1 || nnz_local < 4096) return PCR_OK;
        hipStream_t sd = nullptr;
        HIPCHK(hipStreamCreateWithFlags(&sd, hipStreamNonBlocking));
        hipEvent_t e0, e1, ef, ej;
        HIPCHK(hipEventCreate(&e0)); HIPCHK(hipEventCreate(&e1));
        HIPCHK(hipEventCreateWithFlags(&ef, hipEventDisableTiming)); HIPCHK(hipEventCreateWithFlags(&ej, hipEventDisableTiming));
        const int tile = sddmm_tile ? sddmm_tile : 64, ngrp = 256 / geo.G, span = ngrp * tile;
        Bin &ba = sbins[0], &bb = sbins[1];
        const int na = (int)ba.users.size(), nb = (int)bb.users.size(), rsa = ba.max_lev + 2, rsb = bb.max_lev + 2;
        const bool two = !sh.ws;
        const size_t wb = (vsweep_wave_bytes<T>(ba.cap, rsa, two) + 15) & ~(size_t)15;
        const size_t lds = std::max(wb * 8, small_common(512) + vsweep_bytes<T>(bb.cap, rsb, two));
        const bool dense = lds <= (size_t)40 * 1024;
        const int bc = sweep_pf4 ? 2 : 0;
        auto sddmm = [&](hipStream_t q, int64_t z0, int64_t z1) {
            hipLaunchKernelGGL((k_sddmm<T, 256>), dim3((unsigned)cdiv(z1 - z0, span)), dim3(256), (size_t)span * 8, q, d_U.p, d_p.p, d_ruser.p + z0, d_sitem.p + z0, z1 - z0,
                               d_b.p + z0, geo, tile, (const int*)nullptr, (const int32_t*)nullptr, (const int2*)nullptr, (const int32_t*)nullptr);
        };
        auto sweep = [&](hipStream_t q, int a0, int a1, int b0, int b1) {
            const int grid = (b1 - b0) + cdiv(a1 - a0, 8);
            if (dense) hipLaunchKernelGGL((k_vsweep_all<T, true, 512, 8>), dim3(grid), dim3(512), lds, q, sh, ba.d_users.p + a0, a1 - a0, ba.cap, rsa, wb, bb.d_users.p + b0, b1 - b0, bb.cap, rsb, b1 - b0, d_b.p, d_c.p, strict(), (const int*)nullptr, bc);
            else hipLaunchKernelGGL((k_vsweep_all<T, true, 512, 1>), dim3(grid), dim3(512), lds, q, sh, ba.d_users.p + a0, a1 - a0, ba.cap, rsa, wb, bb.d_users.p + b0, b1 - b0, bb.cap, rsb, b1 - b0, d_b.p, d_c.p, strict(), (const int*)nullptr, bc);
        };
        auto spmm = [&](hipStream_t q, int w0, int w1) {
            hipLaunchKernelGGL((k_spmm<T, 256>), dim3(w1 - w0), dim3(256), 0, q, d_c.p, d_c2r.p, d_cuf.p, d_chunk_ptr.p, d_slot_base.p, d_slot_id.p, d_blk_chunks.p + w0, d_U.p, d_slab.p, geo, (const int*)nullptr);
        };
        auto fin = [&](hipStream_t q) {
            hipLaunchKernelGGL((k_spmm_fin<T, 256, false>), dim3(fin_blocks()), dim3(256), 0, q, d_slab.p, d_item_slot.p, d_p.p, 0.0, (int)d2, d_Hp.p, geo, (const int*)nullptr, (const T*)nullptr, (double*)nullptr, 0);
        };
        const int64_t zh = nnz_local / 2;
        const int wh = (spmm_blocks / 2) & ~7;
        const int R = 60;
        auto timed = [&](const char* what, auto body) -> int {
            float best = 1e30f;
            for (int rep = 0; rep < 3; ++rep) {
                HIPCHK(hipStreamSynchronize(st)); HIPCHK(hipStreamSynchronize(sd));
                HIPCHK(hipEventRecord(e0, st));
                for (int i = 0; i < R; ++i) body();
                HIPCHK(hipEventRecord(e1, st));
                HIPCHK(hipEventSynchronize(e1));
                HIPCHK(hipStreamSynchronize(sd));
                float ms = 0.f;
                HIPCHK(hipEventElapsedTime(&ms, e0, e1));
                best = std::min(best, ms);
            }
            fprintf(stderr, "[pipe-probe] %-74s %7.2f us per product\n", what, 1e3 * best / R);
            return PCR_OK;
        };
        RC(timed("today: sddmm, sweep, spmm, fin on one stream", [&]() { sddmm(st, 0, nnz_local); sweep(st, 0, na, 0, nb); spmm(st, 0, spmm_blocks); fin(st); }));
        RC(timed("  sddmm alone", [&]() { sddmm(st, 0, nnz_local); }));
        RC(timed("  sddmm, first half of the ratings alone", [&]() { sddmm(st, 0, zh); }));
        RC(timed("  sweep alone", [&]() { sweep(st, 0, na, 0, nb); }));
        RC(timed("  sweep, first half of both user lists (the longest users) alone", [&]() { sweep(st, 0, na / 2, 0, nb / 2); }));
        RC(timed("  spmm alone", [&]() { spmm(st, 0, spmm_blocks); }));
        RC(timed("  spmm, first half of the workgroups alone", [&]() { spmm(st, 0, wh); }));
        RC(timed("  fin alone", [&]() { fin(st); }));
        RC(timed("halves back to back on ONE stream (what the split itself costs)", [&]() {
            sddmm(st, 0, zh); sddmm(st, zh, nnz_local); sweep(st, 0, na / 2, 0, nb / 2); sweep(st, na / 2, na, nb / 2, nb); spmm(st, 0, wh); spmm(st, wh, spmm_blocks); fin(st); }));
        RC(timed("two streams: halves side by side, fork + join per product, fin behind the join", [&]() {
            (void)hipEventRecord(ef, st); (void)hipStreamWaitEvent(sd, ef, 0);
            sddmm(st, 0, zh); sddmm(sd, zh, nnz_local); sweep(st, 0, na / 2, 0, nb / 2); sweep(sd, na / 2, na, nb / 2, nb); spmm(st, 0, wh); spmm(sd, wh, spmm_blocks);
            (void)hipEventRecord(ej, sd); (void)hipStreamWaitEvent(st, ej, 0);
            fin(st); }));
        RC(timed("two streams, the side stream one kernel behind (its sddmm starts with the other half's sweep)", [&]() {
            sddmm(st, 0, zh);
            (void)hipEventRecord(ef, st); (void)hipStreamWaitEvent(sd, ef, 0);
            sweep(st, 0, na / 2, 0, nb / 2); sddmm(sd, zh, nnz_local); spmm(st, 0, wh); sweep(sd, na / 2, na, nb / 2, nb); spmm(sd, wh, spmm_blocks);
            (void)hipEventRecord(ej, sd); (void)hipStreamWaitEvent(st, ej, 0);
            fin(st); }));
        RC(timed("full-size sweep on the side stream beside the full-size sddmm (latency-bound beside bandwidth-bound)", [&]() {
            (void)hipEventRecord(ef, st); (void)hipStreamWaitEvent(sd, ef, 0);
            sddmm(st, 0, nnz_local); sweep(sd, 0, na, 0, nb);
            (void)hipEventRecord(ej, sd); (void)hipStreamWaitEvent(st, ej, 0); }));
        RC(timed("full-size spmm on the side stream beside the full-size sddmm (two bandwidth-bound kernels)", [&]() {
            (void)hipEventRecord(ef, st); (void)hipStreamWaitEvent(sd, ef, 0);
            sddmm(st, 0, nnz_local); spmm(sd, 0, spmm_blocks);
            (void)hipEventRecord(ej, sd); (void)hipStreamWaitEvent(st, ej, 0); }));
        HIPCHK(hipStreamSynchronize(st)); HIPCHK(hipStreamSynchronize(sd));
        (void)hipEventDestroy(e0); (void)hipEventDestroy(e1); (void)hipEventDestroy(ef); (void)hipEventDestroy(ej); (void)hipStreamDestroy(sd);
        return PCR_OK;
    }
#endif
    int compute_Ha(const double* a, double* Ha) override {
        RC(need_sorted());
        RC(upload_mat(a, d2, d_p.p));
#ifdef PCR_PIPE_PROBE
        RC(pipe_probe());
        RC(need_sorted());
#endif
        RC(device_hv(d_p.p, d_Hp.p));
        return download_mat(d_Hp.p, d2, Ha);
    }

    int device_cg(int* iters) {
        const int64_t n = (int64_t)d2 * geo.ld;
        {
            ProfScope ps(&prof, "cg", st);
            hipLaunchKernelGGL((k_cg_init<T>), dim3(ew_blocks), dim3(PCR_EW_BLOCK), 0, st, d_g.p, d_delta.p, d_rr.p, d_p.p, n, ew_per_block, d_partA.p);
            hipLaunchKernelGGL(k_cg_init_fin, dim3(1), dim3(PCR_EW_BLOCK), 0, st, d_partA.p, ew_blocks, d_cgp, prm.cg_tol);
        }
        const int* skip = &d_cgp->done;
        const bool fused_dots = single() && n_rng == 1 && !vblock_nbp;
        const bool exact_rr = prm.cg_tol < 1e-5;
        for (int k = 1; k <= prm.cg_max_iter; ++k) {
            RC(device_hv(d_p.p, d_Hp.p, skip, fused_dots ? d_rr.p : nullptr));
            {
                ProfScope ps(&prof, "cg", st);
                if (!fused_dots) hipLaunchKernelGGL((k_cg_a<T>), dim3(ew_blocks), dim3(PCR_EW_BLOCK), 0, st, d_p.p, d_Hp.p, d_rr.p, n, ew_per_block, d_partA.p, d_cgp);
                if (exact_rr) {
                    hipLaunchKernelGGL((k_cg_bc<T, true>), dim3(ew_blocks), dim3(PCR_EW_BLOCK), 0, st, d_p.p, d_Hp.p, d_rr.p, d_delta.p, n, ew_per_block, fused_dots ? fin_blocks() : ew_blocks, d_partA.p, d_cgp, k, d_partB.p);
                    hipLaunchKernelGGL(k_cg_stop, dim3(1), dim3(PCR_EW_BLOCK), 0, st, d_partB.p, ew_blocks, d_cgp, k);
                } else {
                    hipLaunchKernelGGL((k_cg_bc<T, false>), dim3(ew_blocks), dim3(PCR_EW_BLOCK), 0, st, d_p.p, d_Hp.p, d_rr.p, d_delta.p, n, ew_per_block, fused_dots ? fin_blocks() : ew_blocks, d_partA.p, d_cgp, k, (double*)nullptr);
                }
            }
            HIPCHK(hipGetLastError());
        }
        if (iters) {
            HIPCHK(hipMemcpyAsync(h_cg, d_cgp, sizeof(CGState), hipMemcpyDeviceToHost, st));
            RC(sync_checked());
            *iters = h_cg->iters;
        }
        return PCR_OK;
    }
    int solve_delta(const double* g, double* delta, int* iters) override {
        RC(need_sorted());
        RC(upload_mat(g, d2, d_g.p));
        RC(device_cg(iters));
        return download_mat(d_delta.p, d2, delta);
    }

    int update_V(double* now_obj, int* info) override {
        int cg_iters = 0, tries = 0, accepted = 0;
        if (!have_sorted) RC(launch_prepare(d_V.p));
        double prev_obj = 0.0;
        const bool prev_u = !unorm_valid;
        const double unorm2_before = unorm2;
        if (start_sums_queued) start_sums_queued = false;
        else RC(objective_sums(d_objp.p, d_V.p, prev_u, 4));
        RC(device_gradient());
        const bool cg_sync = !prepare_is_single_launch();
        RC(device_cg(cg_sync ? &cg_iters : nullptr));
        double step = prm.stepsize, obj = prev_obj;
        const int64_t n = (int64_t)d2 * geo.ld;
        for (int it = 0; it < 20; ++it) {
            hipLaunchKernelGGL((k_axpy_out<T>), dim3(cdiv(n, 256)), dim3(256), 0, st, d_Vnew.p, d_V.p, d_delta.p, -step, n);
            RC(launch_prepare(d_Vnew.p));
            RC(full_objective(d_Vnew.p, &obj));
            if (!cg_sync) cg_iters = h_cg->iters;
            if (it == 0) prev_obj = h_scal[4] + prm.lambda * ((prev_u ? h_scal[6] : unorm2_before) + h_scal[5]) / 2.0;
            if (ustep_pending) {
                RC(ustep_finish(&fin_obj, fin_info));
                fin_ready = true;
            }
            ++tries;
            if (obj < prev_obj) {
                std::swap(d_V.p, d_Vnew.p);
                accepted = 1;
                break;
            }
            step /= 2.0;
        }
        state_of_rejected_V = !accepted;
        if (now_obj) *now_obj = obj;
        if (info) { info[0] = cg_iters; info[1] = tries; info[2] = accepted; }
        return PCR_OK;
    }

    bool counters_zeroed = false;
    int counter_words() const { return 4 + 64 + (bar_n + 1) / 2; }
    int zero_counters() {
        if (counters_zeroed) return PCR_OK;
        HIPCHK(hipMemsetAsync(d_counters.p, 0, (size_t)counter_words() * sizeof(unsigned long long), st));
        counters_zeroed = true;
        return PCR_OK;
    }
    int launch_ustep() {
        RC(zero_counters());
        counters_zeroed = false;
        const bool newton = tune.ustep_newton != 0;
        const double* dirp = nullptr;
        if (newton && d_dir.p) {
            HIPCHK(hipMemsetAsync(d_dir.p, 0xFF, d_dir.n * sizeof(double), st));
            if (newton_n > 0) {
                const int ldp = (geo.ld + 15) & ~15;
                ProfScope ps(&prof, "unewton", st, -1, newton_n);
                const int wbcap = newton_bytes<T>(newton_cap, newton_rs, geo.ld, ldp, newton_cap) <= (size_t)80 * 1024 ? newton_cap : 0;
                const size_t lds = newton_bytes<T>(newton_cap, newton_rs, geo.ld, ldp, wbcap);
#ifndef PCR_NO_OPTIONAL_KERNELS
                hipLaunchKernelGGL((k_unewton<T>), dim3(newton_grid), dim3(256), lds, st, sh, geo,
                                   d_newton_users.p, newton_n, d_U.p, d_V.p, prm.lambda, strict(), newton_cap, newton_rs, ldp, d_newton_scratch.p, newton_stride, d_dir.p, wbcap);
#else
                (void)lds;
#endif
                HIPCHK(hipGetLastError());
            }
// ... 80 lines not shown
            }
        }
#endif
        if (now_obj) *now_obj = (uobj_merged ? h_uobj[7] : h_uobj[0]) + prm.lambda / 2.0 * (uobj_merged ? h_uobj[5] : h_uobj[1]);
        const int cb = uobj_merged ? 8 : 4;
        if (h_uobj[cb + 2] != 0.0) { pcr_set_error("k_ustep: a workgroup cluster timed out at a hand-off (members not co-resident?)"); return PCR_ERR_DEVICE; }
        if (info) { info[0] = (int64_t)h_uobj[cb]; info[1] = (int64_t)h_uobj[cb + 1]; }
        ustep_rows += h_uobj[cb + 3];
        return PCR_OK;
    }

    int evaluate(int which, int ndcg_k, double* err, double* ndcg) override {
        if (which != 0 && which != 1) { pcr_set_error("which must be 0 (train) or 1 (test)"); return PCR_ERR_ARG; }
        if (ndcg_k < 1) { pcr_set_error("ndcg_k must be >= 1"); return PCR_ERR_ARG; }
        EvalSet& es = ev[which];
        if (es.idcg_k != ndcg_k) {
            std::vector<double> idcg(n_users), disc(ndcg_k);
            for (int k = 1; k <= ndcg_k; ++k) disc[k - 1] = 1.0 / log2((double)k + 1.0);
            if (es.max_raw_levels <= 64) {
                pcr_parallel_ranges(n_users, pcr_host_threads(), [&](int, int64_t lo, int64_t hi) {
                    for (int64_t u = lo; u < hi; ++u) {
                        const int64_t o = es.h_runofs[u], Tn = es.h_runofs[u + 1] - o - 1;
                        const int64_t nowk = std::min<int64_t>(ndcg_k, es.h_uptr[u + 1] - es.h_uptr[u]);
                        double m = 0.0;
                        int64_t k = 1;
                        for (int64_t l = Tn - 1; l >= 0 && k <= nowk; --l)
                            for (int32_t c = 0; c < es.h_cnt[o + l] && k <= nowk; ++c, ++k) m += es.h_lgain[o + l] / log2((double)k + 1.0);
                        idcg[u] = m;
                    }
                });
            } else
            pcr_parallel_ranges(n_users, pcr_host_threads(), [&](int, int64_t lo, int64_t hi) {
                std::vector<double> tmp;
                for (int64_t u = lo; u < hi; ++u) {
                    tmp.assign(es.h_val.begin() + es.h_uptr[u], es.h_val.begin() + es.h_uptr[u + 1]);
                    const int64_t nowk = std::min<int64_t>(ndcg_k, (int64_t)tmp.size());
                    std::partial_sort(tmp.begin(), tmp.begin() + nowk, tmp.end(), [](double a, double b) { return a > b; });
                    double m = 0.0;
                    for (int64_t k = 1; k <= nowk; ++k) m += (pow(2.0, tmp[k - 1]) - 1.0) / log2((double)k + 1.0);
                    idcg[u] = m;
                }
            });
            if (n_users) HIPCHK(hipMemcpy(es.idcg.p, idcg.data(), n_users * sizeof(double), hipMemcpyHostToDevice));
            RC(es.disc.upload(disc, st));
            HIPCHK(hipStreamSynchronize(st));
            es.idcg_k = ndcg_k;
        }
        {
            const bool fast_eval = es.max_raw_levels <= 64;
            const int64_t* up = which == 0 ? d_uptr.p : es.uptr.p;
            const int32_t* it = which == 0 ? d_item.p : es.item.p;
            auto fn = [&](Bin& b, hipStream_t q) {
                const int nus = (int)b.users.size();
                if (fast_eval && b.big) {
                    const int cap_pad = host_pow2(b.cap), rsc = b.max_lev + 2;
                    const size_t lds2 = small_common(512) + carve_bytes(rsc, 4);
                    hipLaunchKernelGGL((k_eval2<T, 512, true>), dim3(std::min(nus, scratch_blocks)), dim3(512), lds2, q, up, it, es.elvl_p, es.erunofs_p,
                                       es.erunstart_p, es.gain.p, es.idcg.p, es.disc.p, ndcg_k, b.d_users.p, nus, d_U.p, d_V.p, geo, d_out4.p, b.cap, cap_pad,
                                       rsc, d_scratch.p, scratch_stride);
                    return;
                }
                if (fast_eval && !b.big) {
                    const int cap_pad = host_pow2(b.cap), rsc = b.max_lev + 2;
                    const size_t lds2 = small_common(b.block) + eval2_bytes<T>(b.cap, cap_pad, rsc);
#define LE2(BL) hipLaunchKernelGGL((k_eval2<T, BL>), dim3(nus), dim3(BL), lds2, q, up, it, es.elvl_p, es.erunofs_p, es.erunstart_p, es.gain.p, es.idcg.p, es.disc.p, ndcg_k, b.d_users.p, nus, d_U.p, d_V.p, geo, d_out4.p, b.cap, cap_pad, rsc)
                    if (b.block == 64) LE2(64); else if (b.block == 256) LE2(256); else LE2(512);
#undef LE2
                    return;
                }
                const size_t smallb = small_common(b.block) + carve_bytes(b.block / PCR_WAVE + 1, sizeof(T)) + carve_bytes(b.block / PCR_WAVE + 1, 4);
                const size_t lds = smallb + (b.big ? 0 : eval_bytes<T>(b.cap));
                const int grid = b.big ? std::min(nus, scratch_blocks) : nus;
#define LE(BL, BG) hipLaunchKernelGGL((k_eval<T, BL, BG>), dim3(grid), dim3(BL), lds, q, up, it, es.val.p, es.gain.p, es.idcg.p, es.disc.p, ndcg_k, b.d_users.p, nus, d_U.p, d_V.p, geo, d_out4.p, b.cap, d_scratch.p, scratch_stride)
                if (b.big) LE(512, true);
                else if (b.block == 64) LE(64, false);
                else if (b.block == 256) LE(256, false);
                else LE(512, false);
#undef LE
            };
            RC(for_bins(es.bins, "eval", fn));
            const int nb = (int)std::min<int64_t>(512, std::max<int64_t>(1, cdiv(n_users, 2048)));
            const int per = cdiv(std::max<int64_t>(n_users, 1), nb);
            hipLaunchKernelGGL(k_sum4_stage1, dim3(nb), dim3(PCR_EW_BLOCK), 0, st, d_out4.p, n_users, per, d_partA.p);
            hipLaunchKernelGGL(k_fin4, dim3(1), dim3(PCR_EW_BLOCK), 0, st, d_partA.p, nb, d_scal.p + 16);
            HIPCHK(hipGetLastError());
        }
        RC(allreduce_f64(d_scal.p + 16, 4));
        HIPCHK(hipMemcpyAsync(h_scal + 16, d_scal.p + 16, 4 * sizeof(double), hipMemcpyDeviceToHost, st));
        RC(sync_checked());
        if (err) *err = h_scal[16] / h_scal[17];
        if (ndcg) *ndcg = h_scal[18] / h_scal[19];
        return PCR_OK;
    }

    int train(pcr_log_fn log, void* ctx, pcr_iter_stats* hist) override {
        char line[512];
        auto emit = [&](const char* s) { if (log) log(ctx, s); else if (rank == 0) { fputs(s, stdout); fputc('\n', stdout); fflush(stdout); } };
        const bool pp = prm.solver_type == PCR_SOLVER_PCRPP;
        snprintf(line, sizeof line, "running %s ndcg_k is %d", pp ? "PrimalCR++" : "PrimalCR", prm.ndcg_k); emit(line);
        snprintf(line, sizeof line, "using %d threads. ", prm.threads); emit(line);
        pcr_iter_stats cur;
        memset(&cur, 0, sizeof cur);
        auto do_eval = [&](pcr_iter_stats& rec) -> int {
            if (!prm.do_predict) return PCR_OK;
            RC(evaluate(0, prm.ndcg_k, &rec.train_err, &rec.train_ndcg));
            snprintf(line, sizeof line, "(Training) pairwise error is %g and ndcg is %g", rec.train_err, rec.train_ndcg); emit(line);
            if (tnnz_file != 0) {
                RC(evaluate(1, prm.ndcg_k, &rec.test_err, &rec.test_ndcg));
                snprintf(line, sizeof line, "(Testing) pairwise error is %g and ndcg is %g", rec.test_err, rec.test_ndcg); emit(line);
            }
            return PCR_OK;
        };
        double now_obj = 0.0;
        RC(launch_prepare(d_V.p));
        RC(full_objective(d_V.p, &now_obj));
        cur.obj = now_obj;
        snprintf(line, sizeof line, "Iter 0 time 0 obj %g", now_obj); emit(line);
        RC(do_eval(cur));
        if (hist) hist[0] = cur;
        if (!prm.do_predict && !log) {
            return iterate(prm.maxiter, hist ? hist + 1 : nullptr, [&](int iter, const pcr_iter_stats& rec) {
                snprintf(line, sizeof line, "Iter %d time %g obj %g", iter, rec.seconds, rec.obj); emit(line);
            });
        }
        double total_time = 0.0;
        for (int iter = 1; iter <= prm.maxiter; ++iter) {
            auto t0 = std::chrono::steady_clock::now();
            int vinfo[3] = {0, 0, 0};
            int64_t uinfo[2] = {0, 0};
            RC(update_V(&now_obj, vinfo));
            RC(update_U(&now_obj, uinfo));
            HIPCHK(hipStreamSynchronize(st));
            total_time += std::chrono::duration<double>(std::chrono::steady_clock::now() - t0).count();
            memset(&cur, 0, sizeof cur);
            cur.obj = now_obj; cur.seconds = total_time;
            cur.cg_v = vinfo[0]; cur.ls_v = vinfo[1]; cur.cg_u = uinfo[0]; cur.ls_u = uinfo[1];
            snprintf(line, sizeof line, "Iter %d time %g obj %g", iter, total_time, now_obj); emit(line);
            RC(do_eval(cur));
            if (hist) hist[iter] = cur;
        }
        return PCR_OK;
    }

    template <class F>
    int iterate(int n, pcr_iter_stats* out, F on_done) {
        if (n <= 0) return PCR_OK;
        hipEvent_t ev0 = nullptr, evk[2] = {nullptr, nullptr};
        HIPCHK(hipEventCreate(&ev0)); HIPCHK(hipEventCreate(&evk[0])); HIPCHK(hipEventCreate(&evk[1]));
        struct Guard { hipEvent_t* e[3]; ~Guard() { for (auto p : e) if (*p) (void)hipEventDestroy(*p); } } guard{{&ev0, &evk[0], &evk[1]}};
        std::vector<pcr_iter_stats> rec(n + 1);
        for (auto& r : rec) memset(&r, 0, sizeof r);
        int rc = PCR_OK;
        device_join = tune.pipeline != 0;
        HIPCHK(hipEventRecord(ev0, st));
        auto close = [&](int k) -> int {
            float ms = 0.f;
            HIPCHK(hipEventElapsedTime(&ms, ev0, evk[k & 1]));
            rec[k].obj = fin_obj; rec[k].seconds = ms / 1e3; rec[k].cg_u = fin_info[0]; rec[k].ls_u = fin_info[1];
            fin_ready = false;
            if (out) out[k - 1] = rec[k];
            on_done(k, rec[k]);
            return PCR_OK;
        };
        const int pipe = tune.pipeline;
        for (int k = 1; k <= n && rc == PCR_OK; ++k) {
            int vinfo[3] = {0, 0, 0};
            double vobj = 0.0;
// ... 285 lines not shown
```

primalcr_amd/csrc/pcr_vside.h:

```cpp
#pragma once
#include "pcr_prims.h"

template <typename T, int BLOCK>
__global__ __launch_bounds__(BLOCK) void k_sddmm(const T* __restrict__ U, const T* __restrict__ M,
                                                 const int32_t* __restrict__ ruser, const int32_t* __restrict__ rows,
                                                 int64_t nnz, T* __restrict__ out, Geo geo, int tile, const int* skip,
                                                 const int32_t* __restrict__ perm, const int2* __restrict__ blk_map,
                                                 const int32_t* __restrict__ chunk_ptr) {
    typedef typename VecOf<T>::type V;
    constexpr int VEC = VecOf<T>::N;
    extern __shared__ __attribute__((aligned(16))) char smem[];
    if (skip && *skip) return;
    const int G = geo.G, g = threadIdx.x & (G - 1), grp = threadIdx.x / G, ngrp = BLOCK / G;
    const int span = ngrp * tile;
    int32_t* s_row = reinterpret_cast<int32_t*>(smem);
    int32_t* s_usr = s_row + span;
    int64_t b0 = (int64_t)blockIdx.x * span;
    int nb = (int)((nnz - b0 < span) ? (nnz - b0) : span);
    if (blk_map) {
        const int2 bc = blk_map[blockIdx.x];
        if (bc.y == 0) return;
        b0 = chunk_ptr[bc.x];
        nb = chunk_ptr[bc.x + bc.y] - (int)b0;
    }
// ... 118 lines not shown
        }
        for (int l = tid; l <= nlev; l += BLOCK) rs[l] = S.runstart[S.runofs[u] + l];
        const int npad = next_pow2(n);
        const bool may_prev = !BIG && sizeof(T) == 4 && S.resort_d > 0 && S.prev_valid;
        const bool from_prev = may_prev && S.rhint[u] != 1;
#pragma unroll 4
        for (int p = tid; p < n; p += BLOCK) {
            if (from_prev) { const unsigned idx = (unsigned)S.sidx[s0 + p]; li[p] = LiOps<LI>::pack(S.slvl[s0 + p], idx); key[p] = m_in[s0 + idx]; }
            else { li[p] = LiOps<LI>::pack(S.lvl[s0 + p], (unsigned)p); key[p] = m_in[s0 + p]; }
        }
        bsync<BLOCK>();
        PPROF(0);
        bool resorted = false;
        if constexpr (!BIG && sizeof(T) == 4)
            if (from_prev)
                resorted = resort_window<T, LI, BLOCK>(key, li, [&](int p) { return (int)LiOps<LI>::lev(li[p]); }, rs, n, reinterpret_cast<int*>(Sx),
                                                       reinterpret_cast<T*>(reinterpret_cast<int*>(Sx) + n), S.resort_d, reinterpret_cast<int*>(red));
        if (!resorted) bitonic_sort<T, LI, BLOCK, false, !BIG>(key, li, npad, n);
        if (may_prev && tid == 0) S.rhint[u] = from_prev ? (resorted ? 0 : 1) : 2;
        PPROF(1);
        for (int p = tid; p < n; p += BLOCK) {
            const LI x = li[p];
            const unsigned idx = LiOps<LI>::idx(x);
            S.ms[s0 + p] = key[p];
            S.slvl[s0 + p] = (uint16_t)LiOps<LI>::lev(x);
            S.sitem[s0 + p] = S.item[s0 + idx];
            S.sidx[s0 + p] = (int32_t)idx;
        }
        PPROF(2);
        double loss;
        if (S.ws) {
            for (int p = tid; p < n; p += BLOCK)
                store_windows<T>(S, (size_t)s0 + p, key, rs, nlev, (int)LiOps<LI>::lev(li[p]), key[p], strict);
            PPROF(3);
            auto levf = [&](int p) { return (int)LiOps<LI>::lev(li[p]); };
            loss = S.w16 ? block_objective_win<T, BLOCK>(key, levf, rs, nlev, n, reinterpret_cast<const uint16_t*>(S.win) + (size_t)s0 * S.ws, S.ws, Sx, red)
                         : block_objective_win<T, BLOCK>(key, levf, rs, nlev, n, reinterpret_cast<const uint32_t*>(S.win) + (size_t)s0 * S.ws, S.ws, Sx, red);
        } else {
            loss = block_objective<T, BLOCK>(key, [&](int p) { return (int)LiOps<LI>::lev(li[p]); }, rs, nlev, n, Sx, red, strict);
        }
        if (tid == 0) S.objp[u] = loss;
        bsync<BLOCK>();
        PPROF(4);
    }
#ifdef PCR_PREP_PROF
    if (tid == 0) {
        const int cls = BLOCK == 64 ? 0 : BLOCK == 256 ? 1 : BIG ? 3 : 2;
        for (int i = 0; i < 5; ++i) atomicAdd(&g_prep_prof[cls * 8 + i], (unsigned long long)pp_[i]);
        atomicAdd(&g_prep_prof[cls * 8 + 7], 1ull);
    }
#endif
}
template <typename T, int BLOCK, bool BIG>
__global__ __launch_bounds__(BLOCK) void k_prepare(Shard<T> S, Geo geo, const int32_t* __restrict__ users, int nusers,
                                                   const T* __restrict__ m_in,
                                                   int cap, int cap_pad, int rs_cap, char* scratch, size_t stride, int strict) {
    extern __shared__ __attribute__((aligned(16))) char smem[];
    prepare_body<T, BLOCK, BIG>(smem, S, users, nusers, m_in, cap, cap_pad, rs_cap, scratch, stride, strict, (int)blockIdx.x, (int)gridDim.x);
}

template <typename T, int WB>
__global__ __launch_bounds__(WB) void k_prepare_all(Shard<T> S, const int32_t* __restrict__ users_a, int nusers_a, int cap_a,
                                                     int cap_pad_a, int rs_cap_a, size_t wave_bytes,
                                                     const int32_t* __restrict__ users_b, int nusers_b, int cap_b, int cap_pad_b,
                                                     int rs_cap_b, int nblk_b, const T* __restrict__ m_in, int strict) {
    extern __shared__ __attribute__((aligned(16))) char smem[];
    if ((int)blockIdx.x < nblk_b)
        prepare_body<T, WB, false>(smem, S, users_b, nusers_b, m_in, cap_b, cap_pad_b, rs_cap_b, nullptr, 0, strict,
                                   (int)blockIdx.x, nblk_b);
    else
        prepare_body<T, 64, false>(smem + (size_t)(threadIdx.x >> 6) * wave_bytes, S, users_a, nusers_a, m_in, cap_a, cap_pad_a,
                                   rs_cap_a, nullptr, 0, strict, ((int)blockIdx.x - nblk_b) * (WB / 64) + (int)(threadIdx.x >> 6),
                                   ((int)gridDim.x - nblk_b) * (WB / 64));
}

template <typename T>
static inline size_t vsweep_bytes(int cap, int rs_cap, bool two) {
    return carve_bytes(cap, sizeof(T)) * (two ? 2 : 1) + carve_bytes(cap + 1, 8) + carve_bytes(rs_cap, 4);
}

template <typename T, int BLOCK, bool BIG, bool HV, bool WT = false>
__device__ __forceinline__ void vsweep_block_body(char* smem, const Shard<T>& S, const int32_t* __restrict__ users, int nusers,
                                                  const T* __restrict__ bsrc, T* __restrict__ c_out, int cap, int rs_cap,
                                                  char* scratch, size_t stride, int strict, int blk, int nblk, int flags = 0) {
    const int b_csr = flags & 1, pf4 = flags & 2;
    Carver small(smem);
    double* red = small.take<double>(BLOCK / PCR_WAVE + 1);
    Carver big(BIG ? scratch + (size_t)blk * stride : small.p);
    T* ms = big.take<T>(cap);
    T* x = (HV && !S.ws) ? big.take<T>(cap) : ms;
    double* Sx = big.take<double>(cap + 1);
    int* rs = big.take<int>(rs_cap);
    const int tid = threadIdx.x;

    for (int ui = blk; ui < nusers; ui += nblk) {
        const int u = users[ui];
        const int64_t s0 = S.uptr[u];
        const int n = (int)(S.uptr[u + 1] - s0);
        const int nlev = (int)(S.runofs[u + 1] - S.runofs[u]) - 1;
        if (n == 0) continue;
        double cu = 1.0;
        if constexpr (WT) cu = S.uw[u];
        if (!HV || !S.ws) {
#pragma unroll 4
            for (int p = tid; p < n; p += BLOCK) ms[p] = S.ms[s0 + p];
        }
        for (int l = tid; l <= nlev; l += BLOCK) rs[l] = S.runstart[S.runofs[u] + l];
        const T* xs = ms;
        if (HV) {
#pragma unroll 4
            for (int p = tid; p < n; p += BLOCK) x[p] = bsrc[s0 + (b_csr ? S.sidx[s0 + p] : p)];
            xs = x;
        }
        __syncthreads();
        block_excl_scan<BLOCK>([&](int i) { return (double)xs[i]; }, Sx, n, red);
        if (S.ws == 4 && S.w16 && pf4) { sweep_out4<T, BLOCK, HV, WT>(S, s0, n, nlev, tid, xs, Sx, rs, c_out, cu); __syncthreads(); continue; }
        for (int p = tid; p < n; p += BLOCK) {
            const int lev = S.slvl[s0 + p];
            const double c = S.ws
                ? sweep_coeff_cached<T>(S, (size_t)(s0 + p), Sx, rs, nlev, lev, (double)xs[p], HV ? 0.0 : 1.0)
                : sweep_coeff<T>(ms, Sx, rs, nlev, lev, ms[p], (double)xs[p], HV ? 0.0 : 1.0, strict);
            c_out[s0 + S.sidx[s0 + p]] = (T)(WT ? c * cu : c);
        }
        __syncthreads();
    }
}
template <typename T, int BLOCK, bool BIG, bool HV, bool WT = false>
__global__ __launch_bounds__(BLOCK) void k_vsweep(Shard<T> S, Geo geo, const int32_t* __restrict__ users, int nusers,
                                                  const T* __restrict__ bsrc, T* __restrict__ c_out,
                                                  int cap, int rs_cap, char* scratch, size_t stride, int strict, const int* skip,
                                                  int b_csr) {
    extern __shared__ __attribute__((aligned(16))) char smem[];
    if (skip && *skip) return;
    vsweep_block_body<T, BLOCK, BIG, HV, WT>(smem, S, users, nusers, bsrc, c_out, cap, rs_cap, scratch, stride, strict,
                                         (int)blockIdx.x, (int)gridDim.x, b_csr);
}

template <typename T>
static inline size_t vsweep_wave_bytes(int cap, int rs_cap, bool two) {
    return carve_bytes(cap, sizeof(T)) * (two ? 2 : 1) + carve_bytes(cap + 1, 8) + carve_bytes(rs_cap, 4);
}
template <typename T, bool HV, bool WT = false>
__device__ __forceinline__ void vsweep_wave_body(char* smem, const Shard<T>& S, const int32_t* __restrict__ users, int nusers,
                                                 const T* __restrict__ bsrc, T* __restrict__ c_out,
                                                 int cap, int rs_cap, size_t wave_bytes, int strict, int ui, int flags = 0) {
    const int b_csr = flags & 1, pf4 = flags & 2;
    const int lane = threadIdx.x & 63, wid = threadIdx.x >> 6;
    if (ui >= nusers) return;
    Carver big(smem + (size_t)wid * wave_bytes);
    T* ms = big.take<T>(cap);
    T* x = (HV && !S.ws) ? big.take<T>(cap) : ms;
    double* Sx = big.take<double>(cap + 1);
    int* rs = big.take<int>(rs_cap);
    const int u = users[ui];
    const int64_t s0 = S.uptr[u];
    const int n = (int)(S.uptr[u + 1] - s0);
    const int nlev = (int)(S.runofs[u + 1] - S.runofs[u]) - 1;
    if (n == 0) return;
    double cu = 1.0;
    if constexpr (WT) cu = S.uw[u];
    if (!HV || !S.ws) {
#pragma unroll 4
        for (int p = lane; p < n; p += 64) ms[p] = S.ms[s0 + p];
    }
    for (int l = lane; l <= nlev; l += 64) rs[l] = S.runstart[S.runofs[u] + l];
    const T* xs = ms;
    if (HV) {
#pragma unroll 4
        for (int p = lane; p < n; p += 64) x[p] = bsrc[s0 + (b_csr ? S.sidx[s0 + p] : p)];
        xs = x;
    }
    wave_sync();
    double carry = 0.0;
    for (int base = 0; base < n; base += 64) {
        const int i = base + lane;
        const double v = (i < n) ? (double)xs[i] : 0.0;
        const double inc = wave_incl_scan(v);
        if (i < n) Sx[i] = carry + inc - v;
        carry += lane63(inc);
    }
    if (lane == 0) Sx[n] = carry;
    wave_sync();
    if (S.ws == 4 && S.w16 && pf4) { sweep_out4<T, 64, HV, WT>(S, s0, n, nlev, lane, xs, Sx, rs, c_out, cu); return; }
    for (int p = lane; p < n; p += 64) {
        const int lev = S.slvl[s0 + p];
        const double c = S.ws
            ? sweep_coeff_cached<T>(S, (size_t)(s0 + p), Sx, rs, nlev, lev, (double)xs[p], HV ? 0.0 : 1.0)
            : sweep_coeff<T>(ms, Sx, rs, nlev, lev, ms[p], (double)xs[p], HV ? 0.0 : 1.0, strict);
        c_out[s0 + S.sidx[s0 + p]] = (T)(WT ? c * cu : c);
    }
}
template <typename T, bool HV, bool WT = false>
__global__ __launch_bounds__(256) void k_vsweep_wave(Shard<T> S, const int32_t* __restrict__ users, int nusers,
                                                     const T* __restrict__ bsrc, T* __restrict__ c_out,
                                                     int cap, int rs_cap, size_t wave_bytes, int strict, const int* skip, int b_csr) {
    extern __shared__ __attribute__((aligned(16))) char smem[];
    if (skip && *skip) return;
    vsweep_wave_body<T, HV, WT>(smem, S, users, nusers, bsrc, c_out, cap, rs_cap, wave_bytes, strict,
                            (int)blockIdx.x * 4 + (int)(threadIdx.x >> 6), b_csr);
}

template <typename T, bool HV, int WB, int MINW = 1, bool WT = false>
__global__ __launch_bounds__(WB, MINW) void k_vsweep_all(Shard<T> S, const int32_t* __restrict__ users_a, int nusers_a, int cap_a,
                                                    int rs_cap_a, size_t wave_bytes, const int32_t* __restrict__ users_b,
                                                    int nusers_b, int cap_b, int rs_cap_b, int nblk_b,
                                                    const T* __restrict__ bsrc, T* __restrict__ c_out, int strict, const int* skip, int b_csr) {
    extern __shared__ __attribute__((aligned(16))) char smem[];
    if (skip && *skip) return;
    if ((int)blockIdx.x < nblk_b)
        vsweep_block_body<T, WB, false, HV, WT>(smem, S, users_b, nusers_b, bsrc, c_out, cap_b, rs_cap_b, nullptr, 0, strict,
                                            (int)blockIdx.x, nblk_b, b_csr);
    else
        vsweep_wave_body<T, HV, WT>(smem, S, users_a, nusers_a, bsrc, c_out, cap_a, rs_cap_a, wave_bytes, strict,
                                ((int)blockIdx.x - nblk_b) * (WB / 64) + (int)(threadIdx.x >> 6), b_csr);
}

template <typename T, int BLOCK>
__global__ __launch_bounds__(BLOCK) void k_spmm(const T* __restrict__ c, const int32_t* __restrict__ c2r,
                                                const int32_t* __restrict__ cuf,
                                                const int32_t* __restrict__ chunk_ptr, const int32_t* __restrict__ inc_base,
                                                const int32_t* __restrict__ slot_id, const int2* __restrict__ blk_chunks,
                                                const T* __restrict__ U, T* __restrict__ slab, Geo geo, const int* skip) {
    typedef typename VecOf<T>::type V;
    constexpr int VEC = VecOf<T>::N;
    if (skip && *skip) return;
    const int G = geo.G, g = threadIdx.x & (G - 1);
    const int2 bc = blk_chunks[blockIdx.x];
    if ((int)threadIdx.x / G >= bc.y) return;
    const int gid = bc.x + (int)threadIdx.x / G;
    const int64_t z0 = chunk_ptr[gid], z1 = chunk_ptr[gid + 1];
    for (int k = 0; k * G < geo.nchunk; ++k) {
        const int ch = g + k * G;
        const bool act = ch < geo.nchunk;
        T acc[VEC];
#pragma unroll
        for (int e = 0; e < VEC; ++e) acc[e] = (T)0;
        int inc = inc_base[gid];
        auto flush = [&]() {
            if (act) {
                V o;
                T* op = reinterpret_cast<T*>(&o);
#pragma unroll
                for (int e = 0; e < VEC; ++e) { op[e] = (T)acc[e]; acc[e] = (T)0; }
                {
                    typedef T nat __attribute__((ext_vector_type(VEC)));
                    nat ov;
#pragma unroll
                    for (int e = 0; e < VEC; ++e) ov[e] = op[e];
                    __builtin_nontemporal_store(ov, reinterpret_cast<nat*>(slab + row_off(slot_id[inc], geo) + ch * VEC));
                }
            }
            inc += 1;
        };
        for (int64_t zb = z0; zb < z1; zb += G) {
            const int64_t zi = zb + g;
            T cr = (T)0;
            int ur = 0;
            if (zi < z1) { cr = c2r ? c[c2r[zi]] : c[zi]; ur = cuf[zi]; }
            const int cnt = (int)((z1 - zb < G) ? (z1 - zb) : G);
            for (int q = 0; q < cnt; q += PCR_UNR) {
                V rv[PCR_UNR];
                T cc[PCR_UNR];
                int uf[PCR_UNR];
#pragma unroll
                for (int e8 = 0; e8 < PCR_UNR; ++e8) {
                    if (q + e8 < cnt) {
                        cc[e8] = __shfl(cr, q + e8, G);
                        uf[e8] = __shfl(ur, q + e8, G);
                        if (act) rv[e8] = *reinterpret_cast<const V*>(U + row_off(uf[e8] & 0x7fffffff, geo) + ch * VEC);
                    }
                }
#pragma unroll
                for (int e8 = 0; e8 < PCR_UNR; ++e8) {
                    if (q + e8 < cnt) {
                        if (uf[e8] < 0) flush();
                        if (act) {
#pragma unroll
                            for (int e = 0; e < VEC; ++e) acc[e] += cc[e8] * velem(rv[e8], e);
                        }
                    }
                }
            }
        }
        flush();
    }
}

template <typename T, int BLOCK, bool DOTS>
__global__ __launch_bounds__(BLOCK) void k_spmm_fin(const T* __restrict__ slab, const int32_t* __restrict__ item_slot,
                                                    const T* __restrict__ base, double beta, int d2, T* __restrict__ out,
                                                    Geo geo, const int* skip, const T* __restrict__ rr, double* __restrict__ part,
                                                    int j0 = 0) {
    typedef typename VecOf<T>::type V;
    constexpr int VEC = VecOf<T>::N;
    __shared__ double red[BLOCK / PCR_WAVE + 1];
    if (skip && *skip) return;
    const int G = geo.G, g = threadIdx.x & (G - 1), ipb = BLOCK / G;
    double x = 0.0, y = 0.0, z = 0.0, w = 0.0;
    for (int j = j0 + (int)blockIdx.x * ipb + (int)threadIdx.x / G; j < d2; j += (int)gridDim.x * ipb) {
        const int s0 = item_slot[j], s1 = item_slot[j + 1];
        for (int ch = g; ch < geo.nchunk; ch += G) {
            double acc[VEC];
            const V bv = *reinterpret_cast<const V*>(base + row_off(j, geo) + ch * VEC);
#pragma unroll
            for (int e = 0; e < VEC; ++e) acc[e] = beta * (double)velem(bv, e);
            for (int sl = s0; sl < s1; sl += 8) {
                V pv[8];
#pragma unroll
                for (int q = 0; q < 8; ++q)
                    if (sl + q < s1) pv[q] = *reinterpret_cast<const V*>(slab + row_off(sl + q, geo) + ch * VEC);
#pragma unroll
                for (int q = 0; q < 8; ++q)
                    if (sl + q < s1) {
#pragma unroll
                        for (int e = 0; e < VEC; ++e) acc[e] += (double)velem(pv[q], e);
                    }
            }
            V o;
            T* op = reinterpret_cast<T*>(&o);
#pragma unroll
            for (int e = 0; e < VEC; ++e) op[e] = (T)acc[e];
            *reinterpret_cast<V*>(out + row_off(j, geo) + ch * VEC) = o;
            if (DOTS) {
                const V rv = *reinterpret_cast<const V*>(rr + row_off(j, geo) + ch * VEC);
#pragma unroll
                for (int e = 0; e < VEC; ++e) {
                    const double pe = (double)velem(bv, e), he = (double)op[e], re = (double)velem(rv, e);
                    x += pe * he;
                    y += re * pe;
                    z += re * he;
                    w += he * he;
                }
            }
        }
    }
    if (DOTS) {
        x = block_sum<BLOCK>(x, red);
        y = block_sum<BLOCK>(y, red);
        z = block_sum<BLOCK>(z, red);
        w = block_sum<BLOCK>(w, red);
        if (threadIdx.x == 0) { part[4 * blockIdx.x] = x; part[4 * blockIdx.x + 1] = y; part[4 * blockIdx.x + 2] = z; part[4 * blockIdx.x + 3] = w; }
    }
}

__global__ void k_spin(long long ticks) {
    const long long t0 = wall_clock64();
    for (int i = 0; i < (1 << 22) && wall_clock64() - t0 < ticks; ++i) __builtin_amdgcn_s_sleep(16);
}
__global__ void k_nop() {}

struct CGState {
    double g2, err, pHp, rp, alpha, rr2, rHp, beta;
    double rr2buf[2];
    int done, iters;
    int done_at, pad_;
};

template <typename T>
__global__ void k_axpy_out(T* __restrict__ out, const T* __restrict__ a, const T* __restrict__ b, double s, int64_t n) {
    const int64_t i = (int64_t)blockIdx.x * blockDim.x + threadIdx.x;
    if (i < n) out[i] = (T)((double)a[i] + s * (double)b[i]);
}

__device__ __forceinline__ void reduce_partials2(const double* part, int nblk, double* a, double* b, double* red) {
    double x = 0.0, y = 0.0;
    for (int i = threadIdx.x; i < nblk; i += PCR_EW_BLOCK) { x += part[2 * i]; y += part[2 * i + 1]; }
    x = block_sum<PCR_EW_BLOCK>(x, red);
    y = block_sum<PCR_EW_BLOCK>(y, red);
    *a = x; *b = y;
}

template <typename T>
__global__ __launch_bounds__(PCR_EW_BLOCK) void k_dots(const T* __restrict__ a, const T* __restrict__ b, int64_t n,
                                                        int per_block, double* __restrict__ part) {
    __shared__ double red[PCR_EW_BLOCK / PCR_WAVE + 1];
    const int64_t lo = (int64_t)blockIdx.x * per_block;
    const int64_t hi = (lo + per_block < n) ? lo + per_block : n;
    double x = 0.0, y = 0.0;
    for (int64_t i = lo + threadIdx.x; i < hi; i += PCR_EW_BLOCK) {
        const double av = (double)a[i];
        x += av * av;
        if (b) y += av * (double)b[i];
    }
    x = block_sum<PCR_EW_BLOCK>(x, red);
    y = block_sum<PCR_EW_BLOCK>(y, red);
    if (threadIdx.x == 0) { part[2 * blockIdx.x] = x; part[2 * blockIdx.x + 1] = y; }
}

__global__ __launch_bounds__(PCR_EW_BLOCK) void k_fin2(const double* __restrict__ part, int nblk, double* __restrict__ out) {
    __shared__ double red[PCR_EW_BLOCK / PCR_WAVE + 1];
    double a, b;
    reduce_partials2(part, nblk, &a, &b, red);
    if (threadIdx.x == 0) { out[0] = a; out[1] = b; }
}

__global__ __launch_bounds__(PCR_EW_BLOCK) void k_sum_stage1(const double* __restrict__ in, int64_t n, int per_block,
                                                              double* __restrict__ part) {
    __shared__ double red[PCR_EW_BLOCK / PCR_WAVE + 1];
    const int64_t lo = (int64_t)blockIdx.x * per_block;
    const int64_t hi = (lo + per_block < n) ? lo + per_block : n;
    double x = 0.0;
    for (int64_t i = lo + threadIdx.x; i < hi; i += PCR_EW_BLOCK) x += in[i];
    x = block_sum<PCR_EW_BLOCK>(x, red);
    if (threadIdx.x == 0) { part[2 * blockIdx.x] = x; part[2 * blockIdx.x + 1] = 0.0; }
}

template <typename T>
__global__ __launch_bounds__(PCR_EW_BLOCK) void k_cg_init(const T* __restrict__ g, T* __restrict__ delta, T* __restrict__ rr,
                                                           T* __restrict__ p, int64_t n,
                                                           int per_block, double* __restrict__ part) {
    __shared__ double red[PCR_EW_BLOCK / PCR_WAVE + 1];
    const int64_t lo = (int64_t)blockIdx.x * per_block;
    const int64_t hi = (lo + per_block < n) ? lo + per_block : n;
    double x = 0.0;
    for (int64_t i = lo + threadIdx.x; i < hi; i += PCR_EW_BLOCK) {
        const T gv = g[i];
        delta[i] = (T)0;
        rr[i] = -gv;
        p[i] = gv;
        x += (double)gv * (double)gv;
    }
    x = block_sum<PCR_EW_BLOCK>(x, red);
    if (threadIdx.x == 0) { part[2 * blockIdx.x] = x; part[2 * blockIdx.x + 1] = 0.0; }
}

__global__ __launch_bounds__(PCR_EW_BLOCK) void k_cg_init_fin(const double* __restrict__ part, int nblk, CGState* st, double tol) {
    __shared__ double red[PCR_EW_BLOCK / PCR_WAVE + 1];
    double a, b;
    reduce_partials2(part, nblk, &a, &b, red);
    if (threadIdx.x == 0) {
        st->g2 = a;
        st->err = sqrt(a) * tol;
        st->done = 0;
        st->iters = 0;
        st->done_at = 0;
        st->rr2buf[0] = a;
    }
}

template <typename T>
__global__ __launch_bounds__(PCR_EW_BLOCK) void k_cg_a(const T* __restrict__ p, const T* __restrict__ Hp, const T* __restrict__ rr,
                                                        int64_t n, int per_block, double* __restrict__ part,
                                                        CGState* st) {
    __shared__ double red[PCR_EW_BLOCK / PCR_WAVE + 1];
    if (st->done) return;
    const int64_t lo = (int64_t)blockIdx.x * per_block;
    const int64_t hi = (lo + per_block < n) ? lo + per_block : n;
    double x = 0.0, y = 0.0, z = 0.0, w = 0.0;
    for (int64_t i = lo + threadIdx.x; i < hi; i += PCR_EW_BLOCK) {
        const double pv = (double)p[i], h = (double)Hp[i], r = (double)rr[i];
        x += pv * h; y += r * pv; z += r * h; w += h * h;
    }
    x = block_sum<PCR_EW_BLOCK>(x, red);
    y = block_sum<PCR_EW_BLOCK>(y, red);
    z = block_sum<PCR_EW_BLOCK>(z, red);
    w = block_sum<PCR_EW_BLOCK>(w, red);
    if (threadIdx.x == 0) { part[4 * blockIdx.x] = x; part[4 * blockIdx.x + 1] = y; part[4 * blockIdx.x + 2] = z; part[4 * blockIdx.x + 3] = w; }
}

template <typename T, bool EXACT>
__global__ __launch_bounds__(PCR_EW_BLOCK) void k_cg_bc(T* __restrict__ p, const T* __restrict__ Hp, T* __restrict__ rr,
                                                         T* __restrict__ delta, int64_t n, int per_block, int nblk,
                                                         const double* __restrict__ part, CGState* st, int k,
                                                         double* __restrict__ part_rr) {
    __shared__ double red[PCR_EW_BLOCK / PCR_WAVE + 1];
    const int da = st->done_at;
    if (da != 0 && da < k) return;
    double s4[4];
    for (int c = 0; c < 4; ++c) {
        double x = 0.0;
        for (int i = threadIdx.x; i < nblk; i += PCR_EW_BLOCK) x += part[4 * i + c];
        s4[c] = block_sum<PCR_EW_BLOCK>(x, red);
    }
    const double pHp = s4[0], rp = s4[1], rHp0 = s4[2], HpHp = s4[3];
    const double rr2_old = st->rr2buf[(k - 1) & 1];
    const double alpha = -1.0 * rp / pHp;
    double rr2 = rr2_old + 2.0 * alpha * rHp0 + alpha * alpha * HpHp;
    rr2 = rr2 > 0.0 ? rr2 : 0.0;
    const double rHp = rHp0 + alpha * HpHp;
    const bool conv = !EXACT && sqrt(rr2) < st->err;
    const double beta = rHp / pHp;
    const int64_t lo = (int64_t)blockIdx.x * per_block;
    const int64_t hi = (lo + per_block < n) ? lo + per_block : n;
    double x2 = 0.0;
    for (int64_t i = lo + threadIdx.x; i < hi; i += PCR_EW_BLOCK) {
        const double pv = (double)p[i], hv = (double)Hp[i];
        delta[i] = (T)((double)delta[i] + pv * alpha);
        const T rn = (T)((double)rr[i] + hv * alpha);
        rr[i] = rn;
        if (EXACT) x2 += (double)rn * (double)rn;
        if (!conv) p[i] = (T)((double)rn * -1.0 + pv * beta);
    }
    if (EXACT) {
        x2 = block_sum<PCR_EW_BLOCK>(x2, red);
        if (threadIdx.x == 0) { part_rr[2 * blockIdx.x] = x2; part_rr[2 * blockIdx.x + 1] = 0.0; }
    }
    if (blockIdx.x == gridDim.x - 1 && threadIdx.x == 0) {
        st->pHp = pHp; st->rp = rp; st->alpha = alpha; st->rr2 = rr2; st->rHp = rHp; st->beta = beta;
        st->iters += 1;
        if (!EXACT) {
            st->rr2buf[k & 1] = rr2;
            if (conv) { st->done_at = k; st->done = 1; }
        }
    }
}
__global__ __launch_bounds__(PCR_EW_BLOCK) void k_cg_stop(const double* __restrict__ part_rr, int nblk, CGState* st, int k) {
    __shared__ double red[PCR_EW_BLOCK / PCR_WAVE + 1];
    if (st->done) return;
    double a, b;
    reduce_partials2(part_rr, nblk, &a, &b, red);
    if (threadIdx.x == 0) {
        st->rr2 = a; st->rr2buf[k & 1] = a;
        if (sqrt(a) < st->err) { st->done_at = k; st->done = 1; }
    }
}
```

Baseline: 47.90 billion pairs/s.

## Batch block reductions, pack per-user team records, and prefetch CG update operands

```diff
diff --git a/primalcr_amd/csrc/pcr_classes.h b/primalcr_amd/csrc/pcr_classes.h
--- a/primalcr_amd/csrc/pcr_classes.h
+++ b/primalcr_amd/csrc/pcr_classes.h
@@ -23,6 +23,7 @@
     int64_t nnz = 0;
     std::vector<int32_t> users;
     DBuf<int32_t> d_users;
+    DBuf<TeamRec> d_recs;
 };
 static const int BIN_LIMIT[3] = {128, 512, 4096};
 static const int BIN_BLOCK[4] = {64, 256, 512, 512};
diff --git a/primalcr_amd/csrc/pcr_eval.h b/primalcr_amd/csrc/pcr_eval.h
--- a/primalcr_amd/csrc/pcr_eval.h
+++ b/primalcr_amd/csrc/pcr_eval.h
@@ -192,11 +192,11 @@
         if (threadIdx.x == 0) part[4 * blockIdx.x + c] = s;
     }
 }
-template <typename T>
+template <typename T, bool CH>
 __global__ __launch_bounds__(PCR_EW_BLOCK) void k_obj3(const double* __restrict__ objx, const double* __restrict__ objx2, int64_t nx,
                                                         const T* __restrict__ a, int64_t na, const T* __restrict__ b, int64_t nb,
                                                         double* __restrict__ part, const double* __restrict__ wx = nullptr) {
-    __shared__ double red[PCR_EW_BLOCK / PCR_WAVE + 1];
+    __shared__ double red[PCR_EW_RED];
     const int64_t G = gridDim.x, blk = blockIdx.x;
     double s[4] = {0.0, 0.0, 0.0, 0.0};
     { const int64_t per = (nx + G - 1) / G, lo = blk * per, hi = lo + per < nx ? lo + per : nx;
@@ -207,21 +207,33 @@
       for (int64_t i = lo + threadIdx.x; i < hi; i += PCR_EW_BLOCK) { const double v = (double)a[i]; s[1] += v * v; } }
     if (b) { const int64_t per = (nb + G - 1) / G, lo = blk * per, hi = lo + per < nb ? lo + per : nb;
       for (int64_t i = lo + threadIdx.x; i < hi; i += PCR_EW_BLOCK) { const double v = (double)b[i]; s[2] += v * v; } }
-    for (int c = 0; c < 4; ++c) {
-        const double t = block_sum<PCR_EW_BLOCK>(s[c], red);
-        if (threadIdx.x == 0) part[4 * blk + c] = t;
-    }
-}
+    block_sums_as<PCR_EW_BLOCK, 4, CH>(s, red);
+    if (threadIdx.x == 0)
+        for (int c = 0; c < 4; ++c) part[4 * blk + c] = s[c];
+}
+template <bool CH>
 __global__ __launch_bounds__(PCR_EW_BLOCK) void k_fin4(const double* __restrict__ part, int nblk, double* __restrict__ out,
                                                         unsigned long long* cnt = nullptr, double* cnt_out = nullptr, int nzero = 0,
                                                         int keep1 = 1) {
-    __shared__ double red[PCR_EW_BLOCK / PCR_WAVE + 1];
-    for (int c = 0; c < 4; ++c) {
-        double x = 0.0;
-        for (int i = threadIdx.x; i < nblk; i += PCR_EW_BLOCK) x += part[4 * i + c];
-        x = block_sum<PCR_EW_BLOCK>(x, red);
-        if (threadIdx.x == 0) out[c] = (c == 1 && !keep1) ? 0.0 : x;
-    }
+    __shared__ double red[PCR_EW_RED];
+    double s4[4] = {0.0, 0.0, 0.0, 0.0};
+    if (CH) {
+        const double2* part2 = reinterpret_cast<const double2*>(part);
+#pragma unroll 4
+        for (int i = threadIdx.x; i < nblk; i += PCR_EW_BLOCK) {
+            const double2 a = part2[2 * i], b = part2[2 * i + 1];
+            s4[0] += a.x; s4[1] += a.y; s4[2] += b.x; s4[3] += b.y;
+        }
+        block_sums<PCR_EW_BLOCK, 4>(s4, red);
+    } else {
+        for (int c = 0; c < 4; ++c) {
+            double x = 0.0;
+            for (int i = threadIdx.x; i < nblk; i += PCR_EW_BLOCK) x += part[4 * i + c];
+            s4[c] = block_sum<PCR_EW_BLOCK>(x, red);
+        }
+    }
+    if (threadIdx.x == 0)
+        for (int c = 0; c < 4; ++c) out[c] = (c == 1 && !keep1) ? 0.0 : s4[c];
     if (cnt) {
         if (threadIdx.x == 0) { cnt_out[0] = (double)cnt[0]; cnt_out[1] = (double)cnt[1]; cnt_out[2] = (double)cnt[3]; cnt_out[3] = (double)cnt[2]; }
         __syncthreads();
diff --git a/primalcr_amd/csrc/pcr_gram.h b/primalcr_amd/csrc/pcr_gram.h
--- a/primalcr_amd/csrc/pcr_gram.h
+++ b/primalcr_amd/csrc/pcr_gram.h
@@ -19,27 +19,6 @@
     static __device__ __forceinline__ int crow(int j, int l) { return (l >> 4) + 4 * j; }
     static __device__ __forceinline__ int ccol(int l) { return l & 15; }
 };
-
-template <int BLOCK, int NV>
-__device__ __forceinline__ void block_sums(double (&v)[NV], double* red) {
-#pragma unroll
-    for (int i = 0; i < NV; ++i) v[i] = wave_sum(v[i]);
-    if (BLOCK == PCR_WAVE) return;
-    const int wid = threadIdx.x >> 6, lane = threadIdx.x & 63;
-    __syncthreads();
-    if (lane == 0) {
-#pragma unroll
-        for (int i = 0; i < NV; ++i) red[wid * NV + i] = v[i];
-    }
-    __syncthreads();
-#pragma unroll
-    for (int i = 0; i < NV; ++i) {
-        double t = 0.0;
-#pragma unroll
-        for (int w = 0; w < BLOCK / PCR_WAVE; ++w) t += red[w * NV + i];
-        v[i] = t;
-    }
-}
 
 template <typename T>
 __host__ __device__ static inline size_t gram_img_bytes(int cap, int nchp) {
diff --git a/primalcr_amd/csrc/pcr_host.cpp b/primalcr_amd/csrc/pcr_host.cpp
--- a/primalcr_amd/csrc/pcr_host.cpp
+++ b/primalcr_amd/csrc/pcr_host.cpp
@@ -319,7 +319,7 @@
 static std::map<std::string, std::string>& tune_table() { static thread_local std::map<std::string, std::string> t; return t; }
 static const char* const TUNE_KEYS[] = {"ustep_mode", "cluster_k", "cluster_users", "ubins", "ustep_gram", "spmm_tiles", "spmm_chunk", "sddmm_csc",
                                         "lanes", "pipeline", "window_cache", "prepare_merged", "resort_window", "allreduce_chunks", "p2p_ll",
-                                        "p2p_timeout_ms", "p2p_queue_budget", "count_rows", "debug", "win16", "ustep_win_lds", "plan_key64", "ustep_newton", "vblock_users", "recommend_select", "ranks_batch_users", "sample_threads", "rerank_lds", "ridge_form", "nnls_form", "itemfold_table_bytes", "fault_cluster_member", "fault_p2p_skip", "fault_p2p_coarse", nullptr};
+                                        "p2p_timeout_ms", "p2p_queue_budget", "count_rows", "debug", "win16", "ustep_win_lds", "plan_key64", "ustep_newton", "vblock_users", "recommend_select", "vside_chains", "ranks_batch_users", "sample_threads", "rerank_lds", "ridge_form", "nnls_form", "itemfold_table_bytes", "fault_cluster_member", "fault_p2p_skip", "fault_p2p_coarse", nullptr};
 extern "C" int pcr_tune(const char* key, const char* value) {
     if (!key) { pcr_set_error("pcr_tune: null key"); return PCR_ERR_ARG; }
     bool known = false;
diff --git a/primalcr_amd/csrc/pcr_prims.h b/primalcr_amd/csrc/pcr_prims.h
--- a/primalcr_amd/csrc/pcr_prims.h
+++ b/primalcr_amd/csrc/pcr_prims.h
@@ -39,6 +39,32 @@
     const double* ulam = nullptr;
 };
 
+struct TeamRec { uint32_t s0; int32_t n; uint32_t ro_lo; uint32_t hi; };
+static inline bool team_rec_fits(int64_t s0, int64_t n, int64_t ro, int64_t nlev) {
+    return s0 >= 0 && s0 < ((int64_t)1 << 32) && ro >= 0 && ro < ((int64_t)1 << 44) && n >= 0 && n < ((int64_t)1 << 31) && nlev >= -1 && nlev + 1 < (1 << 20);
+}
+static inline TeamRec team_rec(int64_t s0, int64_t n, int64_t ro, int64_t nlev) {
+    return TeamRec{(uint32_t)s0, (int32_t)n, (uint32_t)ro, (uint32_t)(nlev + 1) | (uint32_t)(ro >> 32) << 20};
+}
+struct Team { int64_t s0, ro; int n, nlev; };
+template <typename T>
+__device__ __forceinline__ Team load_team(const Shard<T>& S, const TeamRec* __restrict__ recs, int ui, int u) {
+    Team t;
+    if (recs) {
+        const uint4 r = *reinterpret_cast<const uint4*>(recs + ui);
+        t.s0 = (int64_t)r.x;
+        t.ro = (int64_t)r.z | (int64_t)(r.w >> 20) << 32;
+        t.n = (int)r.y;
+        t.nlev = (int)(r.w & 0xFFFFF) - 1;
+    } else {
+        t.s0 = S.uptr[u];
+        t.n = (int)(S.uptr[u + 1] - t.s0);
+        t.ro = S.runofs[u];
+        t.nlev = (int)(S.runofs[u + 1] - t.ro) - 1;
+    }
+    return t;
+}
+
 
 __device__ __forceinline__ int dpp_xor1(int v) { return __builtin_amdgcn_mov_dpp(v, 0xB1, 0xF, 0xF, true); }
 __device__ __forceinline__ int dpp_xor2(int v) { return __builtin_amdgcn_mov_dpp(v, 0x4E, 0xF, 0xF, true); }
@@ -115,6 +141,35 @@
 #pragma unroll
     for (int w = 0; w < BLOCK / PCR_WAVE; ++w) t += red[w];
     return t;
+}
+
+template <int BLOCK, int NV>
+__device__ __forceinline__ void block_sums(double (&v)[NV], double* red) {
+#pragma unroll
+    for (int i = 0; i < NV; ++i) v[i] = wave_sum(v[i]);
+    if (BLOCK == PCR_WAVE) return;
+    const int wid = threadIdx.x >> 6, lane = threadIdx.x & 63;
+    __syncthreads();
+    if (lane == 0) {
+#pragma unroll
+        for (int i = 0; i < NV; ++i) red[wid * NV + i] = v[i];
+    }
+    __syncthreads();
+#pragma unroll
+    for (int i = 0; i < NV; ++i) {
+        double t = 0.0;
+#pragma unroll
+        for (int w = 0; w < BLOCK / PCR_WAVE; ++w) t += red[w * NV + i];
+        v[i] = t;
+    }
+}
+template <int BLOCK, int NV, bool CH>
+__device__ __forceinline__ void block_sums_as(double (&v)[NV], double* red) {
+    if constexpr (CH) block_sums<BLOCK, NV>(v, red);
+    else {
+#pragma unroll
+        for (int i = 0; i < NV; ++i) v[i] = block_sum<BLOCK>(v[i], red);
+    }
 }
 
 template <int BLOCK, class F>
diff --git a/primalcr_amd/csrc/pcr_solver.hip b/primalcr_amd/csrc/pcr_solver.hip
--- a/primalcr_amd/csrc/pcr_solver.hip
+++ b/primalcr_amd/csrc/pcr_solver.hip
@@ -34,7 +34,7 @@
 struct Tune {
     int lanes = 0, spmm_chunk = 0, spmm_tiles = 0, sddmm_csc = -1, ustep_mode = 0, cluster_k = 4, cluster_users = 0, window_cache = 1,
         prepare_merged = -1, pipeline = 1, debug = 0, fault_cluster_member = 0, ustep_gram = -1, count_rows = 0, allreduce_chunks = 0,
-        resort_window = 8, p2p_ll = 16, p2p_timeout_ms = 20000, p2p_queue_budget = 0, fault_p2p_skip = 0, fault_p2p_coarse = 0, win16 = 1, ustep_win_lds = 1, plan_key64 = 0, ustep_newton = 0, vblock_users = 0, recommend_select = 1;
+        resort_window = 8, p2p_ll = 16, p2p_timeout_ms = 20000, p2p_queue_budget = 0, fault_p2p_skip = 0, fault_p2p_coarse = 0, win16 = 1, ustep_win_lds = 1, plan_key64 = 0, ustep_newton = 0, vblock_users = 0, recommend_select = 1, vside_chains = 1;
     std::string ubins;
     void read() {
         lanes = pcr_tune_int("lanes", 0); spmm_chunk = pcr_tune_int("spmm_chunk", 0); spmm_tiles = pcr_tune_int("spmm_tiles", 0);
@@ -48,10 +48,12 @@
         p2p_timeout_ms = pcr_tune_int("p2p_timeout_ms", 20000); fault_p2p_skip = pcr_tune_int("fault_p2p_skip", 0);
         fault_p2p_coarse = pcr_tune_int("fault_p2p_coarse", 0); p2p_queue_budget = pcr_tune_int("p2p_queue_budget", 0);
         win16 = pcr_tune_int("win16", 1); ustep_win_lds = pcr_tune_int("ustep_win_lds", 1); plan_key64 = pcr_tune_int("plan_key64", 0); ustep_newton = pcr_tune_int("ustep_newton", 0); vblock_users = pcr_tune_int("vblock_users", 0);
-        recommend_select = pcr_tune_int("recommend_select", 1);
+        recommend_select = pcr_tune_int("recommend_select", 1); vside_chains = pcr_tune_int("vside_chains", 1);
         ubins.clear(); pcr_tune_get("ubins", &ubins);
     }
 };
+
+#define PCR_WITH_CH(...) do { if (tune.vside_chains) { constexpr bool CH = true; __VA_ARGS__; } else { constexpr bool CH = false; __VA_ARGS__; } } while (0)
 
 template <typename T>
 struct Solver final : pcr_solver {
@@ -538,6 +540,17 @@
         if (vblock_nbp) sddmm_csc = true;
         return PCR_OK;
     }
+    int upload_sweep_list(Bin& b, const HostShard& H) {
+        RC(b.d_users.upload(b.users, st));
+        std::vector<TeamRec> recs(b.users.size());
+        for (size_t i = 0; i < b.users.size(); ++i) {
+            const int64_t u = b.users[i], s0 = H.uptr[u], n = H.uptr[u + 1] - s0, ro = H.lv.run_ofs[u], nlev = H.lv.run_ofs[u + 1] - ro - 1;
+            if (!team_rec_fits(s0, n, ro, nlev)) { pcr_set_error("a shard of 2^32 ratings or 2^44 level runs: beyond the sweeps' team records"); return PCR_ERR_UNSUPPORTED; }
+            recs[i] = team_rec(s0, n, ro, nlev);
+        }
+        return b.d_recs.upload(recs, st);
+    }
+    const TeamRec* recs_of(const Bin& b, size_t first = 0) const { return tune.vside_chains ? b.d_recs.p + first : nullptr; }
     int setup_vside_classes(const HostShard& H) {
         const int64_t nu = n_users;
         make_bins(H.uptr, nu, &H.lv.run_ofs, bins, H.by_len);
@@ -545,7 +558,7 @@
         const int sweep_wave_cap = pick_sweep_wave_cap<T>(H.uptr, nu, H.by_len, ncu);
         if (tune.debug) fprintf(stderr, "[pcr] sweep wave cap %d\n", sweep_wave_cap);
         make_bins(H.uptr, nu, &H.lv.run_ofs, sbins, H.by_len, {std::min(sweep_wave_cap, 4095), 4096}, {64, 512, 512});
-        for (auto& b : sbins) RC(b.d_users.upload(b.users, st));
+        for (auto& b : sbins) RC(upload_sweep_list(b, H));
         const int prep_wave_cap = 256;
         make_bins(H.uptr, nu, &H.lv.run_ofs, pbins, H.by_len, {prep_wave_cap, 4096}, {64, 512, 512});
         for (auto& b : pbins) RC(b.d_users.upload(b.users, st));
@@ -1014,7 +1027,7 @@
             const int rsc = b.max_lev + 2;
             if (b.block == 64) {
                 const size_t wb = (vsweep_wave_bytes<T>(b.cap, rsc, two) + 15) & ~(size_t)15;
-#define LW(HV, WT) hipLaunchKernelGGL((k_vsweep_wave<T, HV, WT>), dim3(cdiv(nus, 4)), dim3(256), wb * 4, q, sh, b.d_users.p, nus, d_b.p, d_c.p, b.cap, rsc, wb, strict(), skip, bc)
+#define LW(HV, WT) hipLaunchKernelGGL((k_vsweep_wave<T, HV, WT>), dim3(cdiv(nus, 4)), dim3(256), wb * 4, q, sh, b.d_users.p, nus, d_b.p, d_c.p, b.cap, rsc, wb, strict(), skip, bc, recs_of(b))
                 if (hv) { if (wt) LW(true, true); else LW(true, false); } else { if (wt) LW(false, true); else LW(false, false); }
 #undef LW
                 return;
@@ -1023,7 +1036,7 @@
             const size_t lds = small_common(b.block) + (b.big ? 0 : bigb);
             const int grid = b.big ? std::min(nus, scratch_blocks) : nus;
 #define LV(BL, BG, HV) do { if (wt) LVW(BL, BG, HV, true); else LVW(BL, BG, HV, false); } while (0)
-#define LVW(BL, BG, HV, WT) hipLaunchKernelGGL((k_vsweep<T, BL, BG, HV, WT>), dim3(grid), dim3(BL), lds, q, sh, geo, b.d_users.p, nus, d_b.p, d_c.p, b.cap, rsc, d_scratch.p, scratch_stride, strict(), skip, bc)
+#define LVW(BL, BG, HV, WT) hipLaunchKernelGGL((k_vsweep<T, BL, BG, HV, WT>), dim3(grid), dim3(BL), lds, q, sh, geo, b.d_users.p, nus, d_b.p, d_c.p, b.cap, rsc, d_scratch.p, scratch_stride, strict(), skip, bc, recs_of(b))
             if (hv) { if (b.big) LV(512, true, true); else LV(512, false, true); }
             else { if (b.big) LV(512, true, false); else LV(512, false, false); }
 #undef LVW
@@ -1041,7 +1054,7 @@
                 ProfScope ps(&prof, std::string(hv ? "vhv" : "vgrad") + "/all", st, ba.nnz + bb.nnz, (int64_t)(na + nb));
 #define LVA(HV, WBS, MW) do { if (wt) LVAW(HV, WBS, MW, true); else LVAW(HV, WBS, MW, false); } while (0)
 #define LVAW(HV, WBS, MW, WT) hipLaunchKernelGGL((k_vsweep_all<T, HV, WBS, MW, WT>), dim3(grid), dim3(WBS), lds, st, sh, ba.d_users.p, na, ba.cap, rsa, wb, \
-                                        bb.d_users.p, nb, bb.cap, rsb, nb, d_b.p, d_c.p, strict(), skip, bc)
+                                        bb.d_users.p, nb, bb.cap, rsb, nb, d_b.p, d_c.p, strict(), skip, bc, recs_of(ba), recs_of(bb))
                 const bool dense = lds <= (size_t)40 * 1024;
                 if (hv) { if (dense) { LVA(true, 512, 8); } else { LVA(true, 512, 1); } } else { if (dense) { LVA(false, 512, 8); } else { LVA(false, 512, 1); } }
 #undef LVAW
@@ -1066,8 +1079,8 @@
         if (j1 <= j0) return PCR_OK;
         const int grid = n_rng == 1 ? fin_blocks() : (int)std::min<int64_t>(1024, cdiv(j1 - j0, 256 / geo.G));
         ProfScope ps2(&prof, "spmm_fin", st);
-        if (dots_rr) hipLaunchKernelGGL((k_spmm_fin<T, 256, true>), dim3(grid), dim3(256), 0, st, d_slab.p, d_item_slot.p, base, beta, j1, out, geo, skip, dots_rr, d_partA.p, j0);
-        else hipLaunchKernelGGL((k_spmm_fin<T, 256, false>), dim3(grid), dim3(256), 0, st, d_slab.p, d_item_slot.p, base, beta, j1, out, geo, skip, (const T*)nullptr, (double*)nullptr, j0);
+        if (dots_rr) PCR_WITH_CH(hipLaunchKernelGGL((k_spmm_fin<T, 256, true, CH>), dim3(grid), dim3(256), 0, st, d_slab.p, d_item_slot.p, base, beta, j1, out, geo, skip, dots_rr, d_partA.p, j0));
+        else hipLaunchKernelGGL((k_spmm_fin<T, 256, false, false>), dim3(grid), dim3(256), 0, st, d_slab.p, d_item_slot.p, base, beta, j1, out, geo, skip, (const T*)nullptr, (double*)nullptr, j0);
         return PCR_OK;
     }
     int launch_spmm(T* out, const T* base, double beta, const int* skip = nullptr, const T* dots_rr = nullptr) {
@@ -1131,7 +1144,7 @@
         const int nb = (int)std::min<int64_t>(512, std::max<int64_t>(1, cdiv(n, 2048)));
         const int per = cdiv(std::max<int64_t>(n, 1), nb);
         hipLaunchKernelGGL(k_sum_stage1, dim3(nb), dim3(PCR_EW_BLOCK), 0, st, in, n, per, d_partA.p);
-        hipLaunchKernelGGL(k_fin2, dim3(1), dim3(PCR_EW_BLOCK), 0, st, d_partA.p, nb, d_scal.p + slot);
+        PCR_WITH_CH(hipLaunchKernelGGL((k_fin2<CH>), dim3(1), dim3(PCR_EW_BLOCK), 0, st, d_partA.p, nb, d_scal.p + slot));
         HIPCHK(hipGetLastError());
         return PCR_OK;
     }
@@ -1139,7 +1152,7 @@
         const int nb = (int)std::min<int64_t>(512, std::max<int64_t>(1, cdiv(n, 4096)));
         const int per = cdiv(std::max<int64_t>(n, 1), nb);
         hipLaunchKernelGGL((k_dots<T>), dim3(nb), dim3(PCR_EW_BLOCK), 0, st, a, (const T*)nullptr, n, per, d_partB.p);
-        hipLaunchKernelGGL(k_fin2, dim3(1), dim3(PCR_EW_BLOCK), 0, st, d_partB.p, nb, d_scal.p + slot);
+        PCR_WITH_CH(hipLaunchKernelGGL((k_fin2<CH>), dim3(1), dim3(PCR_EW_BLOCK), 0, st, d_partB.p, nb, d_scal.p + slot));
         HIPCHK(hipGetLastError());
         return PCR_OK;
     }
@@ -1156,12 +1169,12 @@
     int objective_sums(const double* objx, const T* Vm, bool with_u, int slot = 0, const double* objx2 = nullptr, bool after_ustep = false) {
         const int64_t nV = (int64_t)d2 * geo.ld, nU = (int64_t)n_users * geo.ld;
         const int nb = (int)std::min<int64_t>(512, std::max<int64_t>(1, cdiv(std::max(nV, nU), 4096)));
-        hipLaunchKernelGGL((k_obj3<T>), dim3(nb), dim3(PCR_EW_BLOCK), 0, st, objx, objx2, n_users, Vm, nV, with_u ? d_U.p : (const T*)nullptr, nU, d_partA.p,
-                           objx == d_objp.p ? sh.uw : (const double*)nullptr);
+        PCR_WITH_CH(hipLaunchKernelGGL((k_obj3<T, CH>), dim3(nb), dim3(PCR_EW_BLOCK), 0, st, objx, objx2, n_users, Vm, nV, with_u ? d_U.p : (const T*)nullptr, nU, d_partA.p,
+                                       objx == d_objp.p ? sh.uw : (const double*)nullptr));
         const bool reduce = !single();
         const int keep1 = (!reduce || rank == 0) ? 1 : 0;
-        if (after_ustep) hipLaunchKernelGGL(k_fin4, dim3(1), dim3(PCR_EW_BLOCK), 0, st, d_partA.p, nb, d_scal.p + slot, d_counters.p, d_scal.p + slot + 4, counter_words(), keep1);
-        else hipLaunchKernelGGL(k_fin4, dim3(1), dim3(PCR_EW_BLOCK), 0, st, d_partA.p, nb, d_scal.p + slot, (unsigned long long*)nullptr, (double*)nullptr, 0, keep1);
+        if (after_ustep) PCR_WITH_CH(hipLaunchKernelGGL((k_fin4<CH>), dim3(1), dim3(PCR_EW_BLOCK), 0, st, d_partA.p, nb, d_scal.p + slot, d_counters.p, d_scal.p + slot + 4, counter_words(), keep1));
+        else PCR_WITH_CH(hipLaunchKernelGGL((k_fin4<CH>), dim3(1), dim3(PCR_EW_BLOCK), 0, st, d_partA.p, nb, d_scal.p + slot, (unsigned long long*)nullptr, (double*)nullptr, 0, keep1));
         HIPCHK(hipGetLastError());
         RC(allreduce_f64(d_scal.p + slot, after_ustep ? 8 : 4));
         return PCR_OK;
@@ -1293,8 +1306,8 @@
         };
         auto sweep = [&](hipStream_t q, int a0, int a1, int b0, int b1) {
             const int grid = (b1 - b0) + cdiv(a1 - a0, 8);
-            if (dense) hipLaunchKernelGGL((k_vsweep_all<T, true, 512, 8>), dim3(grid), dim3(512), lds, q, sh, ba.d_users.p + a0, a1 - a0, ba.cap, rsa, wb, bb.d_users.p + b0, b1 - b0, bb.cap, rsb, b1 - b0, d_b.p, d_c.p, strict(), (const int*)nullptr, bc);
-            else hipLaunchKernelGGL((k_vsweep_all<T, true, 512, 1>), dim3(grid), dim3(512), lds, q, sh, ba.d_users.p + a0, a1 - a0, ba.cap, rsa, wb, bb.d_users.p + b0, b1 - b0, bb.cap, rsb, b1 - b0, d_b.p, d_c.p, strict(), (const int*)nullptr, bc);
+            if (dense) hipLaunchKernelGGL((k_vsweep_all<T, true, 512, 8>), dim3(grid), dim3(512), lds, q, sh, ba.d_users.p + a0, a1 - a0, ba.cap, rsa, wb, bb.d_users.p + b0, b1 - b0, bb.cap, rsb, b1 - b0, d_b.p, d_c.p, strict(), (const int*)nullptr, bc, recs_of(ba, a0), recs_of(bb, b0));
+            else hipLaunchKernelGGL((k_vsweep_all<T, true, 512, 1>), dim3(grid), dim3(512), lds, q, sh, ba.d_users.p + a0, a1 - a0, ba.cap, rsa, wb, bb.d_users.p + b0, b1 - b0, bb.cap, rsb, b1 - b0, d_b.p, d_c.p, strict(), (const int*)nullptr, bc, recs_of(ba, a0), recs_of(bb, b0));
         };
         auto spmm = [&](hipStream_t q, int w0, int w1) {
             hipLaunchKernelGGL((k_spmm<T, 256>), dim3(w1 - w0), dim3(256), 0, q, d_c.p, d_c2r.p, d_cuf.p, d_chunk_ptr.p, d_slot_base.p, d_slot_id.p, d_blk_chunks.p + w0, d_U.p, d_slab.p, geo, (const int*)nullptr);
@@ -1371,7 +1384,7 @@
         {
             ProfScope ps(&prof, "cg", st);
             hipLaunchKernelGGL((k_cg_init<T>), dim3(ew_blocks), dim3(PCR_EW_BLOCK), 0, st, d_g.p, d_delta.p, d_rr.p, d_p.p, n, ew_per_block, d_partA.p);
-            hipLaunchKernelGGL(k_cg_init_fin, dim3(1), dim3(PCR_EW_BLOCK), 0, st, d_partA.p, ew_blocks, d_cgp, prm.cg_tol);
+            PCR_WITH_CH(hipLaunchKernelGGL((k_cg_init_fin<CH>), dim3(1), dim3(PCR_EW_BLOCK), 0, st, d_partA.p, ew_blocks, d_cgp, prm.cg_tol));
         }
         const int* skip = &d_cgp->done;
         const bool fused_dots = single() && n_rng == 1 && !vblock_nbp;
@@ -1380,12 +1393,12 @@
             RC(device_hv(d_p.p, d_Hp.p, skip, fused_dots ? d_rr.p : nullptr));
             {
                 ProfScope ps(&prof, "cg", st);
-                if (!fused_dots) hipLaunchKernelGGL((k_cg_a<T>), dim3(ew_blocks), dim3(PCR_EW_BLOCK), 0, st, d_p.p, d_Hp.p, d_rr.p, n, ew_per_block, d_partA.p, d_cgp);
+                if (!fused_dots) PCR_WITH_CH(hipLaunchKernelGGL((k_cg_a<T, CH>), dim3(ew_blocks), dim3(PCR_EW_BLOCK), 0, st, d_p.p, d_Hp.p, d_rr.p, n, ew_per_block, d_partA.p, d_cgp));
                 if (exact_rr) {
-                    hipLaunchKernelGGL((k_cg_bc<T, true>), dim3(ew_blocks), dim3(PCR_EW_BLOCK), 0, st, d_p.p, d_Hp.p, d_rr.p, d_delta.p, n, ew_per_block, fused_dots ? fin_blocks() : ew_blocks, d_partA.p, d_cgp, k, d_partB.p);
-                    hipLaunchKernelGGL(k_cg_stop, dim3(1), dim3(PCR_EW_BLOCK), 0, st, d_partB.p, ew_blocks, d_cgp, k);
+                    PCR_WITH_CH(hipLaunchKernelGGL((k_cg_bc<T, true, CH>), dim3(ew_blocks), dim3(PCR_EW_BLOCK), 0, st, d_p.p, d_Hp.p, d_rr.p, d_delta.p, n, ew_per_block, fused_dots ? fin_blocks() : ew_blocks, d_partA.p, d_cgp, k, d_partB.p));
+                    PCR_WITH_CH(hipLaunchKernelGGL((k_cg_stop<CH>), dim3(1), dim3(PCR_EW_BLOCK), 0, st, d_partB.p, ew_blocks, d_cgp, k));
                 } else {
-                    hipLaunchKernelGGL((k_cg_bc<T, false>), dim3(ew_blocks), dim3(PCR_EW_BLOCK), 0, st, d_p.p, d_Hp.p, d_rr.p, d_delta.p, n, ew_per_block, fused_dots ? fin_blocks() : ew_blocks, d_partA.p, d_cgp, k, (double*)nullptr);
+                    PCR_WITH_CH(hipLaunchKernelGGL((k_cg_bc<T, false, CH>), dim3(ew_blocks), dim3(PCR_EW_BLOCK), 0, st, d_p.p, d_Hp.p, d_rr.p, d_delta.p, n, ew_per_block, fused_dots ? fin_blocks() : ew_blocks, d_partA.p, d_cgp, k, (double*)nullptr));
                 }
             }
             HIPCHK(hipGetLastError());
@@ -1632,7 +1645,7 @@
             const int nb = (int)std::min<int64_t>(512, std::max<int64_t>(1, cdiv(n_users, 2048)));
             const int per = cdiv(std::max<int64_t>(n_users, 1), nb);
             hipLaunchKernelGGL(k_sum4_stage1, dim3(nb), dim3(PCR_EW_BLOCK), 0, st, d_out4.p, n_users, per, d_partA.p);
-            hipLaunchKernelGGL(k_fin4, dim3(1), dim3(PCR_EW_BLOCK), 0, st, d_partA.p, nb, d_scal.p + 16);
+            PCR_WITH_CH(hipLaunchKernelGGL((k_fin4<CH>), dim3(1), dim3(PCR_EW_BLOCK), 0, st, d_partA.p, nb, d_scal.p + 16, (unsigned long long*)nullptr, (double*)nullptr, 0, 1));
             HIPCHK(hipGetLastError());
         }
         RC(allreduce_f64(d_scal.p + 16, 4));
diff --git a/primalcr_amd/csrc/pcr_vside.h b/primalcr_amd/csrc/pcr_vside.h
--- a/primalcr_amd/csrc/pcr_vside.h
+++ b/primalcr_amd/csrc/pcr_vside.h
@@ -224,7 +224,8 @@
 template <typename T, int BLOCK, bool BIG, bool HV, bool WT = false>
 __device__ __forceinline__ void vsweep_block_body(char* smem, const Shard<T>& S, const int32_t* __restrict__ users, int nusers,
                                                   const T* __restrict__ bsrc, T* __restrict__ c_out, int cap, int rs_cap,
-                                                  char* scratch, size_t stride, int strict, int blk, int nblk, int flags = 0) {
+                                                  char* scratch, size_t stride, int strict, int blk, int nblk, int flags,
+                                                  const TeamRec* __restrict__ recs) {
     const int b_csr = flags & 1, pf4 = flags & 2;
     Carver small(smem);
     double* red = small.take<double>(BLOCK / PCR_WAVE + 1);
@@ -237,9 +238,9 @@
 
     for (int ui = blk; ui < nusers; ui += nblk) {
         const int u = users[ui];
-        const int64_t s0 = S.uptr[u];
-        const int n = (int)(S.uptr[u + 1] - s0);
-        const int nlev = (int)(S.runofs[u + 1] - S.runofs[u]) - 1;
+        const Team tm = load_team(S, recs, ui, u);
+        const int64_t s0 = tm.s0;
+        const int n = tm.n, nlev = tm.nlev;
         if (n == 0) continue;
         double cu = 1.0;
         if constexpr (WT) cu = S.uw[u];
@@ -247,7 +248,7 @@
 #pragma unroll 4
             for (int p = tid; p < n; p += BLOCK) ms[p] = S.ms[s0 + p];
         }
-        for (int l = tid; l <= nlev; l += BLOCK) rs[l] = S.runstart[S.runofs[u] + l];
+        for (int l = tid; l <= nlev; l += BLOCK) rs[l] = S.runstart[tm.ro + l];
         const T* xs = ms;
         if (HV) {
 #pragma unroll 4
@@ -271,11 +272,11 @@
 __global__ __launch_bounds__(BLOCK) void k_vsweep(Shard<T> S, Geo geo, const int32_t* __restrict__ users, int nusers,
                                                   const T* __restrict__ bsrc, T* __restrict__ c_out,
                                                   int cap, int rs_cap, char* scratch, size_t stride, int strict, const int* skip,
-                                                  int b_csr) {
+                                                  int b_csr, const TeamRec* __restrict__ recs) {
     extern __shared__ __attribute__((aligned(16))) char smem[];
     if (skip && *skip) return;
     vsweep_block_body<T, BLOCK, BIG, HV, WT>(smem, S, users, nusers, bsrc, c_out, cap, rs_cap, scratch, stride, strict,
-                                         (int)blockIdx.x, (int)gridDim.x, b_csr);
+                                         (int)blockIdx.x, (int)gridDim.x, b_csr, recs);
 }
 
 template <typename T>
@@ -285,7 +286,8 @@
 template <typename T, bool HV, bool WT = false>
 __device__ __forceinline__ void vsweep_wave_body(char* smem, const Shard<T>& S, const int32_t* __restrict__ users, int nusers,
                                                  const T* __restrict__ bsrc, T* __restrict__ c_out,
-                                                 int cap, int rs_cap, size_t wave_bytes, int strict, int ui, int flags = 0) {
+                                                 int cap, int rs_cap, size_t wave_bytes, int strict, int ui, int flags,
+                                                 const TeamRec* __restrict__ recs) {
     const int b_csr = flags & 1, pf4 = flags & 2;
     const int lane = threadIdx.x & 63, wid = threadIdx.x >> 6;
     if (ui >= nusers) return;
@@ -295,9 +297,9 @@
     double* Sx = big.take<double>(cap + 1);
     int* rs = big.take<int>(rs_cap);
     const int u = users[ui];
-    const int64_t s0 = S.uptr[u];
-    const int n = (int)(S.uptr[u + 1] - s0);
-    const int nlev = (int)(S.runofs[u + 1] - S.runofs[u]) - 1;
+    const Team tm = load_team(S, recs, ui, u);
+    const int64_t s0 = tm.s0;
+    const int n = tm.n, nlev = tm.nlev;
     if (n == 0) return;
     double cu = 1.0;
     if constexpr (WT) cu = S.uw[u];
@@ -305,7 +307,7 @@
 #pragma unroll 4
         for (int p = lane; p < n; p += 64) ms[p] = S.ms[s0 + p];
     }
-    for (int l = lane; l <= nlev; l += 64) rs[l] = S.runstart[S.runofs[u] + l];
+    for (int l = lane; l <= nlev; l += 64) rs[l] = S.runstart[tm.ro + l];
     const T* xs = ms;
     if (HV) {
 #pragma unroll 4
@@ -335,26 +337,28 @@
 template <typename T, bool HV, bool WT = false>
 __global__ __launch_bounds__(256) void k_vsweep_wave(Shard<T> S, const int32_t* __restrict__ users, int nusers,
                                                      const T* __restrict__ bsrc, T* __restrict__ c_out,
-                                                     int cap, int rs_cap, size_t wave_bytes, int strict, const int* skip, int b_csr) {
+                                                     int cap, int rs_cap, size_t wave_bytes, int strict, const int* skip, int b_csr,
+                                                     const TeamRec* __restrict__ recs) {
     extern __shared__ __attribute__((aligned(16))) char smem[];
     if (skip && *skip) return;
     vsweep_wave_body<T, HV, WT>(smem, S, users, nusers, bsrc, c_out, cap, rs_cap, wave_bytes, strict,
-                            (int)blockIdx.x * 4 + (int)(threadIdx.x >> 6), b_csr);
+                            (int)blockIdx.x * 4 + (int)(threadIdx.x >> 6), b_csr, recs);
 }
 
 template <typename T, bool HV, int WB, int MINW = 1, bool WT = false>
 __global__ __launch_bounds__(WB, MINW) void k_vsweep_all(Shard<T> S, const int32_t* __restrict__ users_a, int nusers_a, int cap_a,
                                                     int rs_cap_a, size_t wave_bytes, const int32_t* __restrict__ users_b,
                                                     int nusers_b, int cap_b, int rs_cap_b, int nblk_b,
-                                                    const T* __restrict__ bsrc, T* __restrict__ c_out, int strict, const int* skip, int b_csr) {
+                                                    const T* __restrict__ bsrc, T* __restrict__ c_out, int strict, const int* skip, int b_csr,
+                                                    const TeamRec* __restrict__ recs_a, const TeamRec* __restrict__ recs_b) {
     extern __shared__ __attribute__((aligned(16))) char smem[];
     if (skip && *skip) return;
     if ((int)blockIdx.x < nblk_b)
         vsweep_block_body<T, WB, false, HV, WT>(smem, S, users_b, nusers_b, bsrc, c_out, cap_b, rs_cap_b, nullptr, 0, strict,
-                                            (int)blockIdx.x, nblk_b, b_csr);
+                                            (int)blockIdx.x, nblk_b, b_csr, recs_b);
     else
         vsweep_wave_body<T, HV, WT>(smem, S, users_a, nusers_a, bsrc, c_out, cap_a, rs_cap_a, wave_bytes, strict,
-                                ((int)blockIdx.x - nblk_b) * (WB / 64) + (int)(threadIdx.x >> 6), b_csr);
+                                ((int)blockIdx.x - nblk_b) * (WB / 64) + (int)(threadIdx.x >> 6), b_csr, recs_a);
 }
 
 template <typename T, int BLOCK>
@@ -428,22 +432,24 @@
     }
 }
 
-template <typename T, int BLOCK, bool DOTS>
+template <typename T, int BLOCK, bool DOTS, bool CH>
 __global__ __launch_bounds__(BLOCK) void k_spmm_fin(const T* __restrict__ slab, const int32_t* __restrict__ item_slot,
                                                     const T* __restrict__ base, double beta, int d2, T* __restrict__ out,
                                                     Geo geo, const int* skip, const T* __restrict__ rr, double* __restrict__ part,
                                                     int j0 = 0) {
     typedef typename VecOf<T>::type V;
     constexpr int VEC = VecOf<T>::N;
-    __shared__ double red[BLOCK / PCR_WAVE + 1];
+    __shared__ double red[4 * (BLOCK / PCR_WAVE)];
     if (skip && *skip) return;
     const int G = geo.G, g = threadIdx.x & (G - 1), ipb = BLOCK / G;
-    double x = 0.0, y = 0.0, z = 0.0, w = 0.0;
+    double d4[4] = {0.0, 0.0, 0.0, 0.0};
     for (int j = j0 + (int)blockIdx.x * ipb + (int)threadIdx.x / G; j < d2; j += (int)gridDim.x * ipb) {
         const int s0 = item_slot[j], s1 = item_slot[j + 1];
         for (int ch = g; ch < geo.nchunk; ch += G) {
             double acc[VEC];
             const V bv = *reinterpret_cast<const V*>(base + row_off(j, geo) + ch * VEC);
+            V rv = V{};
+            if (DOTS && CH) rv = *reinterpret_cast<const V*>(rr + row_off(j, geo) + ch * VEC);
 #pragma unroll
             for (int e = 0; e < VEC; ++e) acc[e] = beta * (double)velem(bv, e);
             for (int sl = s0; sl < s1; sl += 8) {
@@ -464,24 +470,21 @@
             for (int e = 0; e < VEC; ++e) op[e] = (T)acc[e];
             *reinterpret_cast<V*>(out + row_off(j, geo) + ch * VEC) = o;
             if (DOTS) {
-                const V rv = *reinterpret_cast<const V*>(rr + row_off(j, geo) + ch * VEC);
+                if (!CH) rv = *reinterpret_cast<const V*>(rr + row_off(j, geo) + ch * VEC);
 #pragma unroll
                 for (int e = 0; e < VEC; ++e) {
                     const double pe = (double)velem(bv, e), he = (double)op[e], re = (double)velem(rv, e);
-                    x += pe * he;
-                    y += re * pe;
-                    z += re * he;
-                    w += he * he;
+                    d4[0] += pe * he;
+                    d4[1] += re * pe;
+                    d4[2] += re * he;
+                    d4[3] += he * he;
                 }
             }
         }
     }
     if (DOTS) {
-        x = block_sum<BLOCK>(x, red);
-        y = block_sum<BLOCK>(y, red);
-        z = block_sum<BLOCK>(z, red);
-        w = block_sum<BLOCK>(w, red);
-        if (threadIdx.x == 0) { part[4 * blockIdx.x] = x; part[4 * blockIdx.x + 1] = y; part[4 * blockIdx.x + 2] = z; part[4 * blockIdx.x + 3] = w; }
+        block_sums_as<BLOCK, 4, CH>(d4, red);
+        if (threadIdx.x == 0) { part[4 * blockIdx.x] = d4[0]; part[4 * blockIdx.x + 1] = d4[1]; part[4 * blockIdx.x + 2] = d4[2]; part[4 * blockIdx.x + 3] = d4[3]; }
     }
 }
 
@@ -504,12 +507,13 @@
     if (i < n) out[i] = (T)((double)a[i] + s * (double)b[i]);
 }
 
+#define PCR_EW_RED (4 * (PCR_EW_BLOCK / PCR_WAVE))
+template <bool CH>
 __device__ __forceinline__ void reduce_partials2(const double* part, int nblk, double* a, double* b, double* red) {
-    double x = 0.0, y = 0.0;
-    for (int i = threadIdx.x; i < nblk; i += PCR_EW_BLOCK) { x += part[2 * i]; y += part[2 * i + 1]; }
-    x = block_sum<PCR_EW_BLOCK>(x, red);
-    y = block_sum<PCR_EW_BLOCK>(y, red);
-    *a = x; *b = y;
+    double s[2] = {0.0, 0.0};
+    for (int i = threadIdx.x; i < nblk; i += PCR_EW_BLOCK) { s[0] += part[2 * i]; s[1] += part[2 * i + 1]; }
+    block_sums_as<PCR_EW_BLOCK, 2, CH>(s, red);
+    *a = s[0]; *b = s[1];
 }
 
 template <typename T>
@@ -529,10 +533,11 @@
     if (threadIdx.x == 0) { part[2 * blockIdx.x] = x; part[2 * blockIdx.x + 1] = y; }
 }
 
+template <bool CH>
 __global__ __launch_bounds__(PCR_EW_BLOCK) void k_fin2(const double* __restrict__ part, int nblk, double* __restrict__ out) {
-    __shared__ double red[PCR_EW_BLOCK / PCR_WAVE + 1];
+    __shared__ double red[PCR_EW_RED];
     double a, b;
-    reduce_partials2(part, nblk, &a, &b, red);
+    reduce_partials2<CH>(part, nblk, &a, &b, red);
     if (threadIdx.x == 0) { out[0] = a; out[1] = b; }
 }
 
@@ -566,10 +571,11 @@
     if (threadIdx.x == 0) { part[2 * blockIdx.x] = x; part[2 * blockIdx.x + 1] = 0.0; }
 }
 
+template <bool CH>
 __global__ __launch_bounds__(PCR_EW_BLOCK) void k_cg_init_fin(const double* __restrict__ part, int nblk, CGState* st, double tol) {
-    __shared__ double red[PCR_EW_BLOCK / PCR_WAVE + 1];
+    __shared__ double red[PCR_EW_RED];
     double a, b;
-    reduce_partials2(part, nblk, &a, &b, red);
+    reduce_partials2<CH>(part, nblk, &a, &b, red);
     if (threadIdx.x == 0) {
         st->g2 = a;
         st->err = sqrt(a) * tol;
@@ -580,58 +586,91 @@
     }
 }
 
-template <typename T>
+template <typename T, bool CH>
 __global__ __launch_bounds__(PCR_EW_BLOCK) void k_cg_a(const T* __restrict__ p, const T* __restrict__ Hp, const T* __restrict__ rr,
                                                         int64_t n, int per_block, double* __restrict__ part,
                                                         CGState* st) {
-    __shared__ double red[PCR_EW_BLOCK / PCR_WAVE + 1];
+    __shared__ double red[PCR_EW_RED];
     if (st->done) return;
     const int64_t lo = (int64_t)blockIdx.x * per_block;
     const int64_t hi = (lo + per_block < n) ? lo + per_block : n;
-    double x = 0.0, y = 0.0, z = 0.0, w = 0.0;
+    double d4[4] = {0.0, 0.0, 0.0, 0.0};
     for (int64_t i = lo + threadIdx.x; i < hi; i += PCR_EW_BLOCK) {
         const double pv = (double)p[i], h = (double)Hp[i], r = (double)rr[i];
-        x += pv * h; y += r * pv; z += r * h; w += h * h;
-    }
-    x = block_sum<PCR_EW_BLOCK>(x, red);
-    y = block_sum<PCR_EW_BLOCK>(y, red);
-    z = block_sum<PCR_EW_BLOCK>(z, red);
-    w = block_sum<PCR_EW_BLOCK>(w, red);
-    if (threadIdx.x == 0) { part[4 * blockIdx.x] = x; part[4 * blockIdx.x + 1] = y; part[4 * blockIdx.x + 2] = z; part[4 * blockIdx.x + 3] = w; }
-}
-
-template <typename T, bool EXACT>
+        d4[0] += pv * h; d4[1] += r * pv; d4[2] += r * h; d4[3] += h * h;
+    }
+    block_sums_as<PCR_EW_BLOCK, 4, CH>(d4, red);
+    if (threadIdx.x == 0) { part[4 * blockIdx.x] = d4[0]; part[4 * blockIdx.x + 1] = d4[1]; part[4 * blockIdx.x + 2] = d4[2]; part[4 * blockIdx.x + 3] = d4[3]; }
+}
+
+#define PCR_CG_HOLD 8
+template <typename T, bool EXACT, bool CH>
 __global__ __launch_bounds__(PCR_EW_BLOCK) void k_cg_bc(T* __restrict__ p, const T* __restrict__ Hp, T* __restrict__ rr,
                                                          T* __restrict__ delta, int64_t n, int per_block, int nblk,
                                                          const double* __restrict__ part, CGState* st, int k,
                                                          double* __restrict__ part_rr) {
-    __shared__ double red[PCR_EW_BLOCK / PCR_WAVE + 1];
+    __shared__ double red[PCR_EW_RED];
     const int da = st->done_at;
+    const int64_t lo = (int64_t)blockIdx.x * per_block;
+    const int64_t hi = (lo + per_block < n) ? lo + per_block : n;
+    const bool held = CH && per_block <= PCR_CG_HOLD * PCR_EW_BLOCK;
+    T hp_[PCR_CG_HOLD], hh_[PCR_CG_HOLD], hr_[PCR_CG_HOLD], hd_[PCR_CG_HOLD];
+    double rr2_old = 0.0, err = 0.0;
+    if (CH) {
+        rr2_old = st->rr2buf[(k - 1) & 1];
+        err = st->err;
+    }
+    if (held) {
+#pragma unroll
+        for (int q = 0; q < PCR_CG_HOLD; ++q) {
+            const int64_t i = lo + threadIdx.x + q * PCR_EW_BLOCK;
+            hp_[q] = hh_[q] = hr_[q] = hd_[q] = (T)0;
+            if (i < hi) { hp_[q] = p[i]; hh_[q] = Hp[i]; hr_[q] = rr[i]; hd_[q] = delta[i]; }
+        }
+    }
     if (da != 0 && da < k) return;
-    double s4[4];
-    for (int c = 0; c < 4; ++c) {
-        double x = 0.0;
-        for (int i = threadIdx.x; i < nblk; i += PCR_EW_BLOCK) x += part[4 * i + c];
-        s4[c] = block_sum<PCR_EW_BLOCK>(x, red);
+    double s4[4] = {0.0, 0.0, 0.0, 0.0};
+    if (CH) {
+        const double2* part2 = reinterpret_cast<const double2*>(part);
+#pragma unroll 4
+        for (int i = threadIdx.x; i < nblk; i += PCR_EW_BLOCK) {
+            const double2 a = part2[2 * i], b = part2[2 * i + 1];
+            s4[0] += a.x; s4[1] += a.y; s4[2] += b.x; s4[3] += b.y;
+        }
+        block_sums<PCR_EW_BLOCK, 4>(s4, red);
+    } else {
+        for (int c = 0; c < 4; ++c) {
+            double x = 0.0;
+            for (int i = threadIdx.x; i < nblk; i += PCR_EW_BLOCK) x += part[4 * i + c];
+            s4[c] = block_sum<PCR_EW_BLOCK>(x, red);
+        }
     }
     const double pHp = s4[0], rp = s4[1], rHp0 = s4[2], HpHp = s4[3];
-    const double rr2_old = st->rr2buf[(k - 1) & 1];
+    if (!CH) rr2_old = st->rr2buf[(k - 1) & 1];
     const double alpha = -1.0 * rp / pHp;
     double rr2 = rr2_old + 2.0 * alpha * rHp0 + alpha * alpha * HpHp;
     rr2 = rr2 > 0.0 ? rr2 : 0.0;
     const double rHp = rHp0 + alpha * HpHp;
-    const bool conv = !EXACT && sqrt(rr2) < st->err;
+    if (!CH && !EXACT) err = st->err;
+    const bool conv = !EXACT && sqrt(rr2) < err;
     const double beta = rHp / pHp;
-    const int64_t lo = (int64_t)blockIdx.x * per_block;
-    const int64_t hi = (lo + per_block < n) ? lo + per_block : n;
     double x2 = 0.0;
-    for (int64_t i = lo + threadIdx.x; i < hi; i += PCR_EW_BLOCK) {
-        const double pv = (double)p[i], hv = (double)Hp[i];
-        delta[i] = (T)((double)delta[i] + pv * alpha);
-        const T rn = (T)((double)rr[i] + hv * alpha);
+    auto upd = [&](int64_t i, T p_i, T h_i, T r_i, T d_i) {
+        const double pv = (double)p_i, hv = (double)h_i;
+        delta[i] = (T)((double)d_i + pv * alpha);
+        const T rn = (T)((double)r_i + hv * alpha);
         rr[i] = rn;
         if (EXACT) x2 += (double)rn * (double)rn;
         if (!conv) p[i] = (T)((double)rn * -1.0 + pv * beta);
+    };
+    if (held) {
+#pragma unroll
+        for (int q = 0; q < PCR_CG_HOLD; ++q) {
+            const int64_t i = lo + threadIdx.x + q * PCR_EW_BLOCK;
+            if (i < hi) upd(i, hp_[q], hh_[q], hr_[q], hd_[q]);
+        }
+    } else {
+        for (int64_t i = lo + threadIdx.x; i < hi; i += PCR_EW_BLOCK) upd(i, p[i], Hp[i], rr[i], delta[i]);
     }
     if (EXACT) {
         x2 = block_sum<PCR_EW_BLOCK>(x2, red);
@@ -646,11 +685,12 @@
         }
     }
 }
+template <bool CH>
 __global__ __launch_bounds__(PCR_EW_BLOCK) void k_cg_stop(const double* __restrict__ part_rr, int nblk, CGState* st, int k) {
-    __shared__ double red[PCR_EW_BLOCK / PCR_WAVE + 1];
+    __shared__ double red[PCR_EW_RED];
     if (st->done) return;
     double a, b;
-    reduce_partials2(part_rr, nblk, &a, &b, red);
+    reduce_partials2<CH>(part_rr, nblk, &a, &b, red);
     if (threadIdx.x == 0) {
         st->rr2 = a; st->rr2buf[k & 1] = a;
         if (sqrt(a) < st->err) { st->done_at = k; st->done = 1; }
```

Result: no change. 48.32 billion pairs/s (median of 6 runs) (+0.9%).
